# facebookresearch/goliath

Measured on AMD Instinct MI355X. Metric: relit views/sec (fwd+bwd) at 2048x1334, 250k Gaussians, higher is better.
Workload: dtype f32; 1 GPU; rgca_config2_envrelight; gaussians=250000, views_per_gpu=8, micro_batches=2, world_size=1, dist_backend=none, rccl_world_size=0, parallelism=view-parallel x1, launch=hip_graph_replay

## Files before the change

### goliath_amd/csrc/gol_raster.h

```cpp
#pragma once
#include <type_traits>

#include "gol_common.h"

namespace {

constexpr int kBatch = 256;
constexpr float kUnA = GOL_UN_A, kUnB = GOL_UN_B;
__device__ __forceinline__ float3 true_conic(float a, float b, float c) { return make_float3(a * kUnA, b * kUnB, c * kUnA); }
#ifdef GOL_EXACT_MATH
__device__ __forceinline__ float exact_sigma(float a, float b, float c, float dx, float dy) {
#pragma clang fp contract(off)
  const float t1 = (a * dx) * dx, t2 = (c * dy) * dy, t3 = (b * dx) * dy;
  const float h = 0.5f * (t1 + t2);
  return h + t3;
}
__device__ __forceinline__ float exact_exp_neg(float s) { return (float)exp(-(double)s); }
__device__ __forceinline__ float exact_next_T(float T, float alpha) {
#pragma clang fp contract(off)
  const float om = 1.f - alpha;
  return T * om;
}
#endif

struct TileCoord { int tile, tx, ty; bool ok; };

__device__ __forceinline__ TileCoord tile_of_block(int bid, int T, int tiles_x) {
  const int tiles_y = T / tiles_x;
  const int xcd = bid & 7, j = bid >> 3;
  TileCoord tc;
  const int row_local = j / tiles_x;
  tc.tx = j - row_local * tiles_x;
  tc.ty = row_local * 8 + xcd;
  tc.ok = tc.ty < tiles_y;
  tc.tile = tc.ty * tiles_x + tc.tx;
  return tc;
}

typedef float f1 __attribute__((ext_vector_type(1)));
typedef float f2 __attribute__((ext_vector_type(2)));
typedef int i1 __attribute__((ext_vector_type(1)));
typedef int i2 __attribute__((ext_vector_type(2)));

template <int PPL> struct Pix;
template <> struct Pix<2> { typedef f2 fv; typedef i2 iv; static constexpr int kWaves = 2; };
template <> struct Pix<1> { typedef f1 fv; typedef i1 iv; static constexpr int kWaves = 4; };

template <int PPL>
__device__ __forceinline__ void wave_rect(int wave, float tile_x0, float tile_y0, float& x0, float& x1, float& y0, float& y1) {
  if (PPL == 2) {
    x0 = tile_x0 + 0.5f; x1 = x0 + 15.f; y0 = tile_y0 + (float)(wave * 8) + 0.5f; y1 = y0 + 7.f;
  } else {
    x0 = tile_x0 + (float)((wave & 1) * 8) + 0.5f; x1 = x0 + 7.f; y0 = tile_y0 + (float)((wave >> 1) * 8) + 0.5f; y1 = y0 + 7.f;
  }
}

template <int PPL>
__device__ __forceinline__ int wave_mask(float gx, float gy, float ca, float cb, float cc, float tau, float ia, float ic,
                                         float exact, float tile_x0, float tile_y0) {
  constexpr int NW = Pix<PPL>::kWaves;
  if (!(tau >= 0.f)) return 0;
  if (exact == 0.f) return (1 << NW) - 1;
  int m = 0;
#pragma unroll
  for (int q = 0; q < NW; ++q) {
    float x0, x1, y0, y1;
    wave_rect<PPL>(q, tile_x0, tile_y0, x0, x1, y0, y1);
    const float ms = gol_min_sigma_rect(gx, gy, ca, cb, cc, ia, ic, x0, x1, y0, y1);
    m |= (ms <= tau) ? (1 << q) : 0;
  }
  return m;
}

template <int PPL>
__device__ __forceinline__ void lane_pixel(int tx, int ty, int wave, int lane, int& j, int& i0) {
  if (PPL == 2) { j = tx * 16 + (lane & 15); i0 = ty * 16 + wave * 8 + (lane >> 4) * 2; }
  else { j = tx * 16 + (wave & 1) * 8 + (lane & 7); i0 = ty * 16 + (wave >> 1) * 8 + (lane >> 3); }
}

struct __attribute__((aligned(16))) StagedRow { float4 a, b; float2 c; float2 pad; };

struct Staged { float4 a, b; float2 c; int mask; };
template <int PPL>
__device__ __forceinline__ Staged stage_entry(const float* __restrict__ records, size_t g, float tile_x0, float tile_y0) {
  const float4* R = reinterpret_cast<const float4*>(records + g * GOL_SPLAT_RECORD);
  const float4 q0 = R[0], q1 = R[1], q2 = R[2], q3 = R[3];
  Staged s;
  s.a = q0;
  s.b = q1;
  s.c = make_float2(q2.x, q2.y);
  const float3 cn = true_conic(q0.z, q0.w, q1.x);
  s.mask = wave_mask<PPL>(q0.x, q0.y, cn.x, cn.y, cn.z, q2.z, q2.w, q3.x, q3.y, tile_x0, tile_y0);
  return s;
}

template <typename V, int P>
__device__ __forceinline__ bool any_live(const V& live) {
  unsigned u = 0u;
#pragma unroll
  for (int q = 0; q < P; ++q) u |= __float_as_uint(live[q]);
  return u != 0u;
}

template <int PPL> using fvec = typename Pix<PPL>::fv;
template <int PPL> using ivec = typename Pix<PPL>::iv;

template <int PPL>
__device__ __forceinline__ void visit_falloff(float ca, float cb, float cc, float dx, const fvec<PPL>& dy, fvec<PPL>& sigma,
                                              fvec<PPL>& e) {
#ifndef GOL_EXACT_MATH
  sigma = (ca * dx * dx + cc * dy * dy) + (cb * dx) * dy;
#pragma unroll
  for (int q = 0; q < PPL; ++q) e[q] = __builtin_amdgcn_exp2f(-sigma[q]);
#else
#pragma unroll
  for (int q = 0; q < PPL; ++q) { sigma[q] = exact_sigma(ca, cb, cc, dx, dy[q]); e[q] = exact_exp_neg(sigma[q]); }
#endif
}

template <int PPL>
__device__ __forceinline__ unsigned long long fwd_step(const fvec<PPL>& sigma, fvec<PPL> alpha, const fvec<PPL>& live,
                                                       const fvec<PPL>& T_cur, fvec<PPL>& vis, fvec<PPL>& next_T,
                                                       bool (&take)[PPL], unsigned long long (&stop)[PPL]) {
  alpha *= live;
  vis = alpha * T_cur;
#ifndef GOL_EXACT_MATH
  next_T = T_cur - vis;
#else
#pragma unroll
  for (int q = 0; q < PPL; ++q) next_T[q] = exact_next_T(T_cur[q], alpha[q]);
#endif
  unsigned long long any_stop = 0ull;
#pragma unroll
  for (int q = 0; q < PPL; ++q) {
    const unsigned long long mc = gol_ballot(!(sigma[q] < 0.f)) & gol_ballot(!(alpha[q] < GOL_ALPHA_FLOOR));
    const unsigned long long ms = gol_ballot(next_T[q] <= GOL_T_STOP);
    take[q] = __builtin_amdgcn_inverse_ballot_w64(mc & ~ms);
    stop[q] = mc & ms;
    any_stop |= stop[q];
  }
  return any_stop;
}

template <int PPL>
__device__ __forceinline__ void fwd_take(const bool (&take)[PPL], const fvec<PPL>& next_T, fvec<PPL>& vis, fvec<PPL>& T_cur) {
#pragma unroll
  for (int q = 0; q < PPL; ++q) vis[q] = take[q] ? vis[q] : 0.f;
#ifndef GOL_EXACT_MATH
  T_cur -= vis;
#else
#pragma unroll
  for (int q = 0; q < PPL; ++q) T_cur[q] = take[q] ? next_T[q] : T_cur[q];
#endif
}

template <int PPL>
__device__ __forceinline__ unsigned long long bwd_taken(float opacity, const fvec<PPL>& e, const fvec<PPL>& sigma, int li,
                                                        const ivec<PPL>& bin_final, fvec<PPL>& alpha,
                                                        unsigned long long (&mv)[PPL]) {
  alpha = opacity * e;
  unsigned long long many = 0ull;
#pragma unroll
  for (int q = 0; q < PPL; ++q) {
    alpha[q] = fminf(GOL_ALPHA_CAP_BWD, alpha[q]);
    mv[q] = gol_ballot(li <= bin_final[q]) & gol_ballot(!(sigma[q] < 0.f)) & gol_ballot(!(alpha[q] < GOL_ALPHA_FLOOR));
    many |= mv[q];
  }
  return many;
}

template <int PPL>
__device__ __forceinline__ void bwd_recur(const unsigned long long (&mv)[PPL], fvec<PPL>& alpha, fvec<PPL>& T_cur,
                                          bool (&v)[PPL], fvec<PPL>& ra, fvec<PPL>& fac) {
#pragma unroll
  for (int q = 0; q < PPL; ++q) {
    v[q] = __builtin_amdgcn_inverse_ballot_w64(mv[q]);
    alpha[q] = v[q] ? alpha[q] : 0.f;
  }
  const fvec<PPL> one_m = 1.f - alpha;
#pragma unroll
  for (int q = 0; q < PPL; ++q) ra[q] = __builtin_amdgcn_rcpf(one_m[q]);
  const fvec<PPL> T_new = T_cur * ra;
  fac = alpha * T_new;
  T_cur = T_new;
}

template <int PPL>
__device__ __forceinline__ void bwd_moments(const fvec<PPL>& e, const fvec<PPL>& w, const fvec<PPL>& T_cur,
                                            const fvec<PPL>& ra, const fvec<PPL>& fac, const fvec<PPL>& tail,
                                            const bool (&v)[PPL], const fvec<PPL>& dy, fvec<PPL>& qsum, fvec<PPL>& gop,
                                            fvec<PPL>& gy, fvec<PPL>& gyy) {
  const fvec<PPL> v_alpha = T_cur * w + ra * (tail - qsum);
  qsum += fac * w;
  gop = e * v_alpha;
#pragma unroll
  for (int q = 0; q < PPL; ++q) gop[q] = v[q] ? gop[q] : 0.f;
  gy = gop * dy;
  gyy = gy * dy;
}
template <int PPL>
__device__ __forceinline__ float lane_sum(const fvec<PPL>& x) {
  float s = x[0];
#pragma unroll
  for (int q = 1; q < PPL; ++q) s += x[q];
  return s;
}

template <int PPL>
__device__ __forceinline__ int wave_last_entry(const ivec<PPL>& bin_final) {
  int wmax = bin_final[0];
#pragma unroll
  for (int q = 1; q < PPL; ++q) wmax = max(wmax, bin_final[q]);
#pragma unroll
  for (int off = 32; off > 0; off >>= 1) wmax = max(wmax, __shfl_xor(wmax, off, 64));
  return __builtin_amdgcn_readfirstlane(wmax);
}

inline int64_t raster_grid(int B, int img_h, int img_w) {
  return (int64_t)B * 8 * (((img_h + 15) / 16 + 7) / 8) * ((img_w + 15) / 16);
}

#define GOL_RASTER_CHECK_DIMS(bytes_per_pixel, too_large_msg)                                                           \
  do {                                                                                                                  \
    GOL_REQUIRE(B >= 0 && N >= 0, "negative size");                                                                     \
    GOL_REQUIRE(block == 16, "only block_width == 16 is implemented (the reference's value, render_gsplat.py:28)");     \
    GOL_REQUIRE(img_h > 0 && img_w > 0, "empty image");                                                                 \
    GOL_REQUIRE(raster_grid(B, img_h, img_w) < (1ll << 31), "too many tiles");                                          \
    GOL_REQUIRE((uint64_t)img_h * (uint64_t)img_w * (uint64_t)(bytes_per_pixel) < (1ull << 32), too_large_msg);         \
  } while (0)

template <typename F>
inline void with_ppl(int ppl, F&& fn) {
  if (ppl == 2) fn(std::integral_constant<int, 2>());
  else fn(std::integral_constant<int, 1>());
}
constexpr std::true_type kYes{}; constexpr std::false_type kNo{};

}
```

### goliath_amd/csrc/raster.hip

```cpp
#include <cstdlib>

#include "gol_raster.h"

namespace {

constexpr int kBgGroup = 4;

template <bool EXTRA, bool LAZY, int PPL>
__global__ __launch_bounds__(64 * Pix<PPL>::kWaves) void raster_fwd_kernel(
    int N, int img_h, int img_w, int planar, int tiles_x, int tiles_y, const int2* __restrict__ tile_bins,
    const int32_t* __restrict__ sorted_ids, int64_t capacity, const float* __restrict__ records,
    const float* __restrict__ background, float* __restrict__ out_img,
    float* __restrict__ out_extra, float* __restrict__ final_Ts, int32_t* __restrict__ final_idx,
    float* __restrict__ out_alpha, float* __restrict__ out_extra_norm, float norm_lo,
    const float* __restrict__ l1_target, const float* __restrict__ l1_mask, int l1_mask_c,
    uint8_t* __restrict__ l1_sign, float* __restrict__ l1_partial, int n_views, int bg_group, int bg_vec16) {
  typedef typename Pix<PPL>::fv fv;
  typedef typename Pix<PPL>::iv iv;
  constexpr int NW = Pix<PPL>::kWaves, NT = 64 * NW;
  __shared__ float s_l1[NW];
  __shared__ float4 s_a[kBatch];
  __shared__ float4 s_b[kBatch];
  __shared__ float2 s_c[kBatch];
  __shared__ int32_t s_mask[kBatch];
  const int T = tiles_x * tiles_y;
  const int view = blockIdx.x % n_views, slot = blockIdx.x / n_views;
  const TileCoord tc = tile_of_block(slot, T, tiles_x);
  if (!tc.ok) return;
  const int tid = threadIdx.x, lane = tid & 63, wave = tid >> 6;

  int2 range;
  auto fill_group = [&](auto g_c) -> bool {
    constexpr int G = decltype(g_c)::value;
    const int tx0 = tc.tx & ~(G - 1), n = min(G, tiles_x - tx0);
    const size_t tile0 = (size_t)view * T + (size_t)(tc.tile - (tc.tx - tx0));
    int entries = 0;
#pragma unroll
    for (int t = 0; t < G; ++t) {
      const int2 r = tile_bins[tile0 + min(t, n - 1)];
      entries |= (r.y > r.x) ? 1 : 0;
      if (t == tc.tx - tx0) range = r;
    }
    if (entries) return false;
    if (tc.tx != tx0) return true;
    const unsigned hw = (unsigned)img_h * (unsigned)img_w;
    const size_t vplane = (size_t)view * hw;
    const float Tq = 1.f, ex = 0.f;
    const float c0 = 0.f + Tq * background[0], c1 = 0.f + Tq * background[1], c2 = 0.f + Tq * background[2];
    const float al = 1.f - Tq;
    const float nrm = ex / fminf(fmaxf(1.f - Tq, norm_lo), 1.f);
    float* __restrict__ o_T = final_Ts + vplane;
    float* __restrict__ o_img = out_img + 3 * vplane;
    float* __restrict__ o_img1 = o_img + hw;
    float* __restrict__ o_img2 = o_img + 2u * hw;
    float* __restrict__ o_ex = (EXTRA && out_extra) ? out_extra + vplane : nullptr;
    float* __restrict__ o_alpha = out_alpha ? out_alpha + vplane : nullptr;
    float* __restrict__ o_norm = (EXTRA && out_extra_norm) ? out_extra_norm + vplane : nullptr;
    const int x0 = tx0 * 16, y0 = tc.ty * 16;
    const int rw = min(x0 + 16 * G, img_w) - x0, nrows = min(16, img_h - y0);
    auto fill_rows = [&](auto v_c) {
      constexpr int V = decltype(v_c)::value;
      typedef float vt __attribute__((ext_vector_type(V)));
      typedef int it __attribute__((ext_vector_type(V)));
      constexpr int CPR = 16 * G / V, RPP = NT / CPR;
      const int col = (tid % CPR) * V, r0 = tid / CPR;
#pragma unroll
      for (int k = 0; k * RPP < 16; ++k) {
        const int r = r0 + k * RPP;
        if (col < rw && r < nrows) {
          const unsigned b4 = ((unsigned)(y0 + r) * (unsigned)img_w + (unsigned)(x0 + col)) * 4u;
          *reinterpret_cast<vt*>(gol_at(o_T, b4)) = vt(Tq);
          if (!LAZY) *reinterpret_cast<it*>(gol_at(final_idx + vplane, b4)) = it(0);
          *reinterpret_cast<vt*>(gol_at(o_img, b4)) = vt(c0);
          *reinterpret_cast<vt*>(gol_at(o_img1, b4)) = vt(c1);
          *reinterpret_cast<vt*>(gol_at(o_img2, b4)) = vt(c2);
          if (o_ex) *reinterpret_cast<vt*>(gol_at(o_ex, b4)) = vt(ex);
          if (o_alpha) *reinterpret_cast<vt*>(gol_at(o_alpha, b4)) = vt(al);
          if (o_norm) *reinterpret_cast<vt*>(gol_at(o_norm, b4)) = vt(nrm);
        }
      }
    };
    if (bg_vec16) fill_rows(std::integral_constant<int, 4>());
    else fill_rows(std::integral_constant<int, 2>());
    if (!l1_target) return true;
    const float* __restrict__ i_tgt = l1_target + 3 * vplane;
    const float* __restrict__ i_mask = l1_mask ? l1_mask + (size_t)l1_mask_c * vplane : nullptr;
    float* s_part = reinterpret_cast<float*>(s_a);
    constexpr int CH = G < 4 ? G : 4;
    auto l1_tiles = [&](auto m_c) {
      constexpr int MC = decltype(m_c)::value;
      const float cs[3] = {c0, c1, c2};
#pragma unroll
      for (int tb = 0; tb < G; tb += CH) {
        if (tb >= n) break;
        float tg[CH][PPL][3], mk[CH][PPL][3];
        bool ok[CH][PPL];
#pragma unroll
        for (int t = 0; t < CH; ++t) {
          int tj, ti0;
          lane_pixel<PPL>(tx0 + tb + t, tc.ty, wave, lane, tj, ti0);
#pragma unroll
          for (int q = 0; q < PPL; ++q) {
            ok[t][q] = (ti0 + q < img_h) && (tj < img_w);
            const unsigned b4 = ((unsigned)min(ti0 + q, img_h - 1) * (unsigned)img_w + (unsigned)min(tj, img_w - 1)) * 4u;
#pragma unroll
            for (int c = 0; c < 3; ++c) {
              tg[t][q][c] = *gol_at(i_tgt + (size_t)c * hw, b4);
              mk[t][q][c] = MC == 0 ? 1.f : (MC == 3 || c == 0) ? *gol_at(i_mask + (size_t)c * hw, b4) : mk[t][q][0];
            }
          }
        }
#pragma unroll
        for (int t = 0; t < CH; ++t) {
          float l1_acc = 0.f;
#pragma unroll
          for (int q = 0; q < PPL; ++q) {
#pragma unroll
            for (int c = 0; c < 3; ++c) {
              const float d = (cs[c] - tg[t][q][c]) * mk[t][q][c];
              l1_acc += ok[t][q] ? fabsf(d) : 0.f;
            }
          }
          const float ws = gol_wave_sum_to_lane63(l1_acc);
          if (lane == 63) s_part[(tb + t) * NW + wave] = ws;
        }
      }
    };
    if (!i_mask) l1_tiles(std::integral_constant<int, 0>());
    else if (l1_mask_c == 3) l1_tiles(std::integral_constant<int, 3>());
    else l1_tiles(std::integral_constant<int, 1>());
    __syncthreads();
    if (tid < n) {
      float tot = 0.f;
#pragma unroll
      for (int w = 0; w < NW; ++w) tot += s_part[tid * NW + w];
      l1_partial[tile0 + tid] = tot;
    }
    return true;
  };
  if (PPL == 2 && bg_group) {
    const bool done = bg_group == 2 ? fill_group(std::integral_constant<int, 2>())
                    : bg_group == 4 ? fill_group(std::integral_constant<int, 4>())
                                    : fill_group(std::integral_constant<int, 8>());
    if (done) return;
  } else {
    range = tile_bins[(size_t)view * T + tc.tile];
  }

  int j, i0;
  lane_pixel<PPL>(tc.tx, tc.ty, wave, lane, j, i0);
  bool in[PPL];
  fv py, live;
#pragma unroll
  for (int q = 0; q < PPL; ++q) {
    in[q] = (i0 + q < img_h) && (j < img_w);
    py[q] = (float)(i0 + q) + 0.5f;
    live[q] = in[q] ? 1.f : 0.f;
  }
  const float px = (float)j + 0.5f;

  const int32_t* ids = sorted_ids + (size_t)view * capacity;
  const size_t goff = (size_t)view * N;

  fv T_cur = 1.f;
  iv cur_idx = 0;
  fv acc0 = 0.f, acc1 = 0.f, acc2 = 0.f, acc3 = 0.f;

  const int n_batches = (range.y - range.x + kBatch - 1) / kBatch;
  for (int bb = 0; bb < n_batches; ++bb) {
    if (__syncthreads_and(!any_live<fv, PPL>(live))) break;
    const int batch_start = range.x + bb * kBatch;
    for (int k = tid; k < kBatch; k += NT) {
      const int idx = batch_start + k;
      if (idx < range.y) {
        const Staged st = stage_entry<PPL>(records, goff + (size_t)ids[idx], (float)(tc.tx * 16), (float)(tc.ty * 16));
        s_a[k] = st.a; s_b[k] = st.b; s_c[k] = st.c; s_mask[k] = st.mask;
      } else {
        s_mask[k] = 0;
      }
    }
    __syncthreads();
    const int batch_size = min(kBatch, range.y - batch_start);
    for (int chunk = 0; chunk < batch_size; chunk += 64) {
      unsigned long long bits = gol_ballot((s_mask[chunk + lane] >> wave) & 1);
      if (LAZY && gol_ballot(any_live<fv, PPL>(live)) == 0ull) break;
      while (bits) {
        if (!LAZY && gol_ballot(any_live<fv, PPL>(live)) == 0ull) { chunk = batch_size; break; }
        const int t = chunk + __builtin_ctzll(bits);
        bits &= bits - 1;
        const float4 a4 = s_a[t];
        const float4 b4 = s_b[t];
        const float2 c2 = s_c[t];
        const float dx = a4.x - px;
        const fv dy = a4.y - py;
        fv sigma, e, alpha, vis, next_T;
        visit_falloff<PPL>(a4.z, a4.w, b4.x, dx, dy, sigma, e);
#pragma unroll
        for (int q = 0; q < PPL; ++q) alpha[q] = fminf(GOL_ALPHA_CAP_FWD, b4.y * e[q]);
        bool take[PPL];
        unsigned long long stop_m[PPL];
        const unsigned long long any_stop = fwd_step<PPL>(sigma, alpha, live, T_cur, vis, next_T, take, stop_m);
        bool half_done = false;
        if (!LAZY || any_stop != 0ull) {
#pragma unroll
          for (int q = 0; q < PPL; ++q) {
            const bool stop = __builtin_amdgcn_inverse_ballot_w64(stop_m[q]);
            live[q] = stop ? 0.f : live[q];
            if (LAZY) cur_idx[q] = stop ? (batch_start + t - 1) : cur_idx[q];
          }
          if (LAZY) half_done = gol_ballot(any_live<fv, PPL>(live)) == 0ull;
        }
        fwd_take<PPL>(take, next_T, vis, T_cur);
        acc0 += b4.z * vis; acc1 += b4.w * vis; acc2 += c2.x * vis;
        if (EXTRA) acc3 += c2.y * vis;
        if (!LAZY) {
#pragma unroll
          for (int q = 0; q < PPL; ++q) cur_idx[q] = take[q] ? (batch_start + t) : cur_idx[q];
        }
        if (LAZY && half_done) { chunk = batch_size; break; }
      }
    }
  }
  if (LAZY) {
#pragma unroll
    for (int q = 0; q < PPL; ++q) cur_idx[q] = live[q] != 0.f ? range.y - 1 : cur_idx[q];
  }

  const unsigned hw = (unsigned)img_h * (unsigned)img_w;
  const size_t vplane = (size_t)view * hw;
  float* __restrict__ o_T = final_Ts + vplane;
  int32_t* __restrict__ o_idx = final_idx + vplane;
  float* __restrict__ o_img = out_img + 3 * vplane;
  float* __restrict__ o_ex = (EXTRA && out_extra) ? out_extra + vplane : nullptr;
  float* __restrict__ o_alpha = out_alpha ? out_alpha + vplane : nullptr;
  float* __restrict__ o_norm = (EXTRA && out_extra_norm) ? out_extra_norm + vplane : nullptr;
  const float* __restrict__ i_tgt = l1_target ? l1_target + 3 * vplane : nullptr;
  const float* __restrict__ i_mask = l1_mask ? l1_mask + (size_t)l1_mask_c * vplane : nullptr;
  uint8_t* __restrict__ o_sign = l1_target ? l1_sign + vplane : nullptr;
  const float bg0 = background[0], bg1 = background[1], bg2 = background[2];
  float* __restrict__ o_img1 = o_img + (planar ? hw : 1u);
  float* __restrict__ o_img2 = o_img + (planar ? 2u * hw : 2u);
  const bool bwd_state = range.y > range.x;
  float l1_acc = 0.f;
#pragma unroll
  for (int q = 0; q < PPL; ++q) {
    if (!in[q]) continue;
    const unsigned pix = (unsigned)(i0 + q) * (unsigned)img_w + (unsigned)j;
    const unsigned b4 = pix * 4u;
    const unsigned bimg = planar ? b4 : 3u * b4;
    const float Tq = T_cur[q];
    const float c0 = acc0[q] + Tq * bg0, c1 = acc1[q] + Tq * bg1, c2 = acc2[q] + Tq * bg2, ex = acc3[q];
    *gol_at(o_T, b4) = Tq;
    if (bwd_state || !LAZY) *gol_at(o_idx, b4) = cur_idx[q];
    *gol_at(o_img, bimg) = c0; *gol_at(o_img1, bimg) = c1; *gol_at(o_img2, bimg) = c2;
    if (o_ex) *gol_at(o_ex, b4) = ex;
    if (o_alpha) *gol_at(o_alpha, b4) = 1.f - Tq;
    if (o_norm) *gol_at(o_norm, b4) = ex / fminf(fmaxf(1.f - Tq, norm_lo), 1.f);
    if (i_tgt) {
      const float m0 = i_mask ? *gol_at(i_mask, b4) : 1.f;
      const float cs[3] = {c0, c1, c2};
      unsigned code = 0u;
#pragma unroll
      for (int c = 0; c < 3; ++c) {
        const float m = (i_mask && l1_mask_c == 3) ? *gol_at(i_mask + (size_t)c * hw, b4) : m0;
        const float d = (cs[c] - *gol_at(i_tgt + (size_t)c * hw, b4)) * m;
        l1_acc += fabsf(d);
        code |= (d > 0.f ? 2u : (d < 0.f ? 0u : 1u)) << (2 * c);
      }
      if (bwd_state) *gol_at(o_sign, pix) = (uint8_t)code;
    }
  }
  if (l1_target) {
    const float ws = gol_wave_sum_to_lane63(l1_acc);
    if (lane == 63) s_l1[wave] = ws;
    __syncthreads();
    if (tid == 0) {
      float tot = 0.f;
#pragma unroll
      for (int w = 0; w < NW; ++w) tot += s_l1[w];
      l1_partial[(size_t)view * T + tc.tile] = tot;
    }
  }
}

__global__ __launch_bounds__(1024) void l1_sum_kernel(int n, const float* __restrict__ l1_partial, float scale,
                                                      float* __restrict__ l1_out) {
  __shared__ float s_w[16];
  float a0 = 0.f, a1 = 0.f, a2 = 0.f, a3 = 0.f;
  const int n4 = n >> 2;
  const float4* p4 = reinterpret_cast<const float4*>(l1_partial);
  int i = threadIdx.x;
  for (; i + 3 * 1024 < n4; i += 4 * 1024) {
    const float4 v0 = p4[i], v1 = p4[i + 1024], v2 = p4[i + 2048], v3 = p4[i + 3072];
    a0 += (v0.x + v0.y) + (v0.z + v0.w); a1 += (v1.x + v1.y) + (v1.z + v1.w);
    a2 += (v2.x + v2.y) + (v2.z + v2.w); a3 += (v3.x + v3.y) + (v3.z + v3.w);
  }
  for (; i < n4; i += 1024) { const float4 v = p4[i]; a0 += (v.x + v.y) + (v.z + v.w); }
  if ((int)threadIdx.x < (n & 3)) a1 += l1_partial[4 * n4 + threadIdx.x];
  const float ws = gol_wave_sum_to_lane63((a0 + a1) + (a2 + a3));
  if ((threadIdx.x & 63) == 63) s_w[threadIdx.x >> 6] = ws;
  __syncthreads();
  if (threadIdx.x == 0) {
    float tot = 0.f;
#pragma unroll
    for (int w = 0; w < 16; ++w) tot += s_w[w];
    l1_out[0] = tot * scale;
  }
}

constexpr int kBatchB = 64;
constexpr int kAcc = 12;

static_assert(kBatchB == 64, "raster_bwd_kernel ballots one 64-entry chunk per batch");

template <bool EXTRA, bool PACKED, int PPL>
__global__ __launch_bounds__(64 * Pix<PPL>::kWaves) void raster_bwd_kernel(
    int N, int img_h, int img_w, int planar, int tiles_x, int tiles_y, const int2* __restrict__ tile_bins,
    const int32_t* __restrict__ sorted_ids, int64_t capacity, const float* __restrict__ records,
    const float* __restrict__ background,
    const float* __restrict__ final_Ts, const int32_t* __restrict__ final_idx,
    const float* __restrict__ v_out_img, const float* __restrict__ v_out_extra,
    const float* __restrict__ v_out_alpha, float* __restrict__ v_xy, float* __restrict__ v_conic,
    float* __restrict__ v_colors, float* __restrict__ v_extra, float* __restrict__ v_opacity,
    const uint8_t* __restrict__ v_sign, const float* __restrict__ v_sign_mask, int v_sign_mask_c,
    const float* __restrict__ v_img_scale, float v_img_scale_mul, int n_views) {
  typedef typename Pix<PPL>::fv fv;
  typedef typename Pix<PPL>::iv iv;
  constexpr int NW = Pix<PPL>::kWaves, NT = 64 * NW;
  __shared__ StagedRow s_e[kBatchB];
  __shared__ int32_t s_mask[kBatchB];
  __shared__ int32_t s_id[kBatchB];
  __shared__ __attribute__((aligned(16))) float s_acc[NW][kBatchB][kAcc];
  __shared__ int32_t s_touched[NW][kBatchB];
  __shared__ int32_t s_wmax[NW];
  const int T = tiles_x * tiles_y;
  const int view = blockIdx.x % n_views, slot = blockIdx.x / n_views;
  const TileCoord tc = tile_of_block(slot, T, tiles_x);
  if (!tc.ok) return;
  const int2 range = tile_bins[(size_t)view * T + tc.tile];
  if (range.y <= range.x) return;
  const int tid = threadIdx.x, lane = tid & 63, wave = tid >> 6;
  int j, i0;
  lane_pixel<PPL>(tc.tx, tc.ty, wave, lane, j, i0);
  const float px = (float)j + 0.5f;
  const size_t hw = (size_t)img_h * img_w;
  const int32_t* ids = sorted_ids + (size_t)view * capacity;
  const size_t goff = (size_t)view * N;
  bool in[PPL];
  size_t pp[PPL];
  fv py, T_final;
  iv bin_final;
#pragma unroll
  for (int q = 0; q < PPL; ++q) {
    in[q] = (i0 + q < img_h) && (j < img_w);
    py[q] = (float)(i0 + q) + 0.5f;
    pp[q] = in[q] ? ((size_t)view * img_h + i0 + q) * img_w + j : 0;
    T_final[q] = in[q] ? final_Ts[pp[q]] : 1.f;
    bin_final[q] = in[q] ? final_idx[pp[q]] : (range.x - 1);
  }
  fv T_cur = T_final;
  fv vo0 = 0.f, vo1 = 0.f, vo2 = 0.f, vo3 = 0.f, voa = 0.f;
  {
    const float vsc = (v_img_scale ? v_img_scale[0] : 1.f) * v_img_scale_mul;
    const size_t os = planar ? hw : 1;
#pragma unroll
    for (int q = 0; q < PPL; ++q) {
      if (!in[q]) continue;
      const size_t p = pp[q];
      const int i = i0 + q;
      const size_t o = planar ? (size_t)view * 3 * hw + (size_t)i * img_w + j : 3 * p;
      float g0 = 0.f, g1 = 0.f, g2 = 0.f;
      if (v_out_img) { g0 = v_out_img[o]; g1 = v_out_img[o + os]; g2 = v_out_img[o + 2 * os]; }
      if (v_sign) {
        const unsigned code = v_sign[p];
        float m0 = vsc, m1 = vsc, m2 = vsc;
        if (v_sign_mask) {
          const float* mk = v_sign_mask + (size_t)view * v_sign_mask_c * hw + (size_t)i * img_w + j;
          m0 *= mk[0]; m1 *= (v_sign_mask_c == 3) ? mk[hw] : mk[0]; m2 *= (v_sign_mask_c == 3) ? mk[2 * hw] : mk[0];
        }
        g0 += (float)((int)(code & 3u) - 1) * m0;
        g1 += (float)((int)((code >> 2) & 3u) - 1) * m1;
        g2 += (float)((int)((code >> 4) & 3u) - 1) * m2;
      }
      vo0[q] = g0; vo1[q] = g1; vo2[q] = g2;
      if (EXTRA && v_out_extra) vo3[q] = v_out_extra[p];
      if (v_out_alpha) voa[q] = v_out_alpha[p];
    }
  }
  const fv tail = T_final * (voa - (background[0] * vo0 + background[1] * vo1 + background[2] * vo2));
  fv qsum = 0.f;

  const int wmax = wave_last_entry<PPL>(bin_final);
  if (lane == 0) s_wmax[wave] = wmax;
  __syncthreads();
  int bmax = s_wmax[0];
#pragma unroll
  for (int w = 1; w < NW; ++w) bmax = max(bmax, s_wmax[w]);
  bmax = min(bmax, range.y - 1);
  if (bmax < range.x) return;

  float* acc_lane = &s_acc[wave][0][lane >> 4];
  const int n_batches = (bmax - range.x + kBatchB) / kBatchB;
  auto entry_id = [&](int bb2) {
    const int e = bmax - bb2 * kBatchB - tid;
    return (tid < kBatchB && e >= range.x) ? ids[e] : 0;
  };
  int gid_next = entry_id(0);
  unsigned rec_bytes = GOL_GRAD_RECORD * sizeof(float);
  if (PACKED) asm volatile("" : "+s"(rec_bytes));
  for (int bb = 0; bb < n_batches; ++bb) {
    __syncthreads();
    const int batch_end = bmax - bb * kBatchB;
    const int batch_size = min(kBatchB, batch_end + 1 - range.x);
    const int gid = gid_next;
    if (tid < kBatchB) {
      if (tid < batch_size) {
        const Staged st = stage_entry<PPL>(records, goff + (size_t)gid, (float)(tc.tx * 16), (float)(tc.ty * 16));
        s_e[tid].a = st.a; s_e[tid].b = st.b; s_e[tid].c = st.c; s_mask[tid] = st.mask;
        s_id[tid] = gid;
      } else {
        s_mask[tid] = 0;
      }
    }
    if (bb + 1 < n_batches) gid_next = entry_id(bb + 1);
    (&s_touched[0][0])[tid] = 0;
    __syncthreads();

    const int t0 = max(0, batch_end - wmax);
    unsigned long long bits = gol_ballot((s_mask[lane] >> wave) & 1);
    if (t0 > 0) bits &= ~0ull << t0;
    while (bits) {
      const int t = __builtin_ctzll(bits);
      bits &= bits - 1;
      const float4 a4 = s_e[t].a;
      const float4 b4 = s_e[t].b;
      const float2 c2 = s_e[t].c;
      const int li = batch_end - t;
      const float dx = a4.x - px;
      const fv dy = a4.y - py;
      fv sigma, vis, alpha, ra, fac;
      visit_falloff<PPL>(a4.z, a4.w, b4.x, dx, dy, sigma, vis);
      unsigned long long mv[PPL];
      if (bwd_taken<PPL>(b4.y, vis, sigma, li, bin_final, alpha, mv) == 0ull) continue;
      bool v[PPL];
      bwd_recur<PPL>(mv, alpha, T_cur, v, ra, fac);
      fv w = b4.z * vo0 + b4.w * vo1 + c2.x * vo2;
      if (EXTRA) w += c2.y * vo3;
      fv gop, gy, gyy;
      bwd_moments<PPL>(vis, w, T_cur, ra, fac, tail, v, dy, qsum, gop, gy, gyy);
      float g0s, g1s, g2s, g3 = 0.f;
      if (PPL == 2) {
        g0s = __builtin_fmaf(fac[0], vo0[0], fac[PPL - 1] * vo0[PPL - 1]);
        g1s = __builtin_fmaf(fac[0], vo1[0], fac[PPL - 1] * vo1[PPL - 1]);
        g2s = __builtin_fmaf(fac[0], vo2[0], fac[PPL - 1] * vo2[PPL - 1]);
        if (EXTRA) g3 = __builtin_fmaf(fac[0], vo3[0], fac[PPL - 1] * vo3[PPL - 1]);
      } else {
        g0s = fac[0] * vo0[0]; g1s = fac[0] * vo1[0]; g2s = fac[0] * vo2[0];
        if (EXTRA) g3 = fac[0] * vo3[0];
      }
      const float m0 = lane_sum<PPL>(gop), my = lane_sum<PPL>(gy), myy = lane_sum<PPL>(gyy);
      const float mx = m0 * dx, mxx = mx * dx, mxy = my * dx;
      const float r0 = gol_wave_sum4(g0s, g1s, g2s, m0);
      const float r1 = gol_wave_sum4(mx, my, mxx, mxy);
      const float r2 = gol_wave_sum_to_lane63(myy);
      const float r3 = EXTRA ? gol_wave_sum_to_lane63(g3) : 0.f;
      if ((lane & 15) == 15) {
        float* a = gol_at(acc_lane, (unsigned)t * (unsigned)(kAcc * sizeof(float)));
        a[0] = r0; a[4] = r1;
        if (lane == 63) { a[8 - 3] = r2; a[9 - 3] = r3; }
        s_touched[wave][t] = 1;
      }
    }
    __syncthreads();
    if (PACKED) {
      if (tid < kBatchB) {
        int tw[NW];
#pragma unroll
        for (int w = 0; w < NW; ++w) tw[w] = s_touched[w][tid];
        float s[kAcc];
#pragma unroll
        for (int k = 0; k < kAcc; ++k) s[k] = 0.f;
        bool any = false;
#pragma unroll
        for (int w = 0; w < NW; ++w) {
          if (tw[w]) {
            any = true;
            const float4* q = reinterpret_cast<const float4*>(&s_acc[w][tid][0]);
            const float4 q0 = q[0], q1 = q[1], q2 = q[2];
            s[0] += q0.x; s[1] += q0.y; s[2] += q0.z; s[3] += q0.w;
            s[4] += q1.x; s[5] += q1.y; s[6] += q1.z; s[7] += q1.w;
            s[8] += q2.x; s[9] += q2.y;
          }
        }
        if (any) {
          const float4 a4 = s_e[tid].a;
          const float4 b4 = s_e[tid].b;
          const float nop = -b4.y, cc = b4.x;
          const float wxx = nop * a4.z * kUnA, wxy = nop * a4.w * kUnB, wyy = nop * cc * kUnA, hnop = 0.5f * nop;
          float4* o = reinterpret_cast<float4*>(&s_acc[0][tid][0]);
          o[0] = make_float4(s[0], s[1], s[2], s[3]);
          o[1] = make_float4(wxx * s[4] + wxy * s[5], wxy * s[4] + wyy * s[5], hnop * s[6], nop * s[7]);
          *reinterpret_cast<float2*>(o + 2) = make_float2(hnop * s[8], s[9]);
          s_touched[0][tid] = 1;
        }
      }
      __syncthreads();
      const int c = tid & 15;
      if (c <= (EXTRA ? 9 : 8)) {
        float* rec_c = v_colors + goff * 16 + c;
        constexpr int kIt = kBatchB * 16 / NT, kCh = 4;
        static_assert(kIt % kCh == 0, "the merge issues its atomics in chunks of kCh entries per lane");
#pragma unroll
        for (int i0 = 0; i0 < kIt; i0 += kCh) {
          int flag[kCh], id[kCh];
          float val[kCh];
#pragma unroll
          for (int i = 0; i < kCh; ++i) {
            const int t = (tid >> 4) + (i0 + i) * (NT / 16);
            flag[i] = s_touched[0][t]; id[i] = s_id[t]; val[i] = s_acc[0][t][c];
          }
#pragma unroll
          for (int i = 0; i < kCh; ++i) {
            if (flag[i]) {
              char* r = reinterpret_cast<char*>(rec_c) + (uint64_t)(unsigned)id[i] * rec_bytes;
              atomicAdd(reinterpret_cast<float*>(r), val[i]);
            }
          }
        }
      }
    } else if (tid < batch_size) {
      float a[kAcc];
#pragma unroll
      for (int k = 0; k < kAcc; ++k) a[k] = 0.f;
      bool any = false;
#pragma unroll
      for (int w = 0; w < NW; ++w) {
        if (s_touched[w][tid]) {
          any = true;
          const float4* q = reinterpret_cast<const float4*>(&s_acc[w][tid][0]);
          const float4 q0 = q[0], q1 = q[1], q2 = q[2];
          a[0] += q0.x; a[1] += q0.y; a[2] += q0.z; a[3] += q0.w;
          a[4] += q1.x; a[5] += q1.y; a[6] += q1.z; a[7] += q1.w;
          a[8] += q2.x; a[9] += q2.y;
        }
      }
      if (any) {
        const size_t g = goff + (size_t)s_id[tid];
        const float4 a4 = s_e[tid].a;
        const float4 b4 = s_e[tid].b;
        const float nop = -b4.y;
        const float3 cn = true_conic(a4.z, a4.w, b4.x);
        atomicAdd(v_colors + 3 * g, a[0]); atomicAdd(v_colors + 3 * g + 1, a[1]); atomicAdd(v_colors + 3 * g + 2, a[2]);
        atomicAdd(v_opacity + g, a[3]);
        atomicAdd(v_xy + 2 * g, nop * (cn.x * a[4] + cn.y * a[5]));
        atomicAdd(v_xy + 2 * g + 1, nop * (cn.y * a[4] + cn.z * a[5]));
        atomicAdd(v_conic + 3 * g, 0.5f * nop * a[6]); atomicAdd(v_conic + 3 * g + 1, nop * a[7]);
        atomicAdd(v_conic + 3 * g + 2, 0.5f * nop * a[8]);
        if (EXTRA && v_extra) atomicAdd(v_extra + g, a[9]);
      }
    }
  }
}

__global__ __launch_bounds__(256) void raster_count_pairs_kernel(int N, int img_h, int img_w, int tiles_x, int tiles_y,
                                                                 const int2* __restrict__ tile_bins,
                                                                 const int32_t* __restrict__ sorted_ids, int64_t capacity,
                                                                 const float* __restrict__ records,
                                                                 const int32_t* __restrict__ final_idx,
                                                                 unsigned long long* __restrict__ counts) {
  __shared__ unsigned long long s_cnt[2];
  const int view = blockIdx.y, tile = blockIdx.x, T = tiles_x * tiles_y;
  const int ty = tile / tiles_x, tx = tile - ty * tiles_x;
  const int j = tx * 16 + (threadIdx.x & 15), i = ty * 16 + (threadIdx.x >> 4);
  if (threadIdx.x < 2) s_cnt[threadIdx.x] = 0ull;
  __syncthreads();
  const int2 range = tile_bins[(size_t)view * T + tile];
  unsigned long long tested = 0, taken = 0;
  if (i < img_h && j < img_w && range.y > range.x) {
    const int last = min(range.y - 1, final_idx[((size_t)view * img_h + i) * img_w + j]);
    const float px = (float)j + 0.5f, py = (float)i + 0.5f;
    for (int li = range.x; li <= last; ++li) {
      const float4* R = reinterpret_cast<const float4*>(records + ((size_t)view * N + sorted_ids[(size_t)view * capacity + li]) * GOL_SPLAT_RECORD);
      const float4 q0 = R[0], q1 = R[1];
      const float dx = q0.x - px, dy = q0.y - py;
      f1 sg, e;
      visit_falloff<1>(q0.z, q0.w, q1.x, dx, f1(dy), sg, e);
      const float alpha = fminf(GOL_ALPHA_CAP_FWD, q1.y * e[0]);
      ++tested;
      taken += (!(sg[0] < 0.f) && !(alpha < GOL_ALPHA_FLOOR)) ? 1 : 0;
    }
  }
  atomicAdd(&s_cnt[0], tested);
  atomicAdd(&s_cnt[1], taken);
  __syncthreads();
  if (threadIdx.x < 2 && s_cnt[threadIdx.x]) atomicAdd(counts + 2 * view + threadIdx.x, s_cnt[threadIdx.x]);
}

__global__ __launch_bounds__(256) void splat_pack_kernel(size_t n, const float* __restrict__ xys,
                                                         const float* __restrict__ conics,
                                                         const float* __restrict__ colors,
                                                         const float* __restrict__ extra,
                                                         const float* __restrict__ opacities,
                                                         float* __restrict__ records) {
  const size_t e = (size_t)blockIdx.x * 256 + threadIdx.x;
  if (e >= n) return;
  gol_record_write(records + e * GOL_SPLAT_RECORD, xys[2 * e], xys[2 * e + 1], conics[3 * e], conics[3 * e + 1],
                   conics[3 * e + 2], opacities[e], colors ? colors[3 * e] : 0.f, colors ? colors[3 * e + 1] : 0.f,
                   colors ? colors[3 * e + 2] : 0.f, extra ? extra[e] : 0.f);
}

}

extern "C" int gol_raster_plan(int B, int* fwd_pixels_per_lane) {
  static const int forced = getenv("GOL_RASTER_PPL") ? atoi(getenv("GOL_RASTER_PPL")) : 0;
  if (fwd_pixels_per_lane) *fwd_pixels_per_lane = (forced == 1 || forced == 2) ? forced : (B <= 2 ? 1 : 2);
  return GOL_OK;
}

extern "C" int gol_raster_count_pairs(int B, int N, int img_h, int img_w, const int32_t* tile_bins, const int32_t* sorted_ids,
                                      int64_t capacity, const float* records, const int32_t* final_idx, uint64_t* counts,
                                      void* stream) {
  GOL_REQUIRE(B >= 0 && N >= 0 && img_h > 0 && img_w > 0, "bad size");
  if (B == 0) return GOL_OK;
  GOL_REQUIRE(tile_bins && final_idx && counts && (capacity == 0 || sorted_ids) && (N == 0 || records), "null pointer");
  hipStream_t s = (hipStream_t)stream;
  if (hipMemsetAsync(counts, 0, sizeof(uint64_t) * 2 * (size_t)B, s) != hipSuccess) {
    gol_set_error("gol_raster_count_pairs: hipMemsetAsync failed");
    return GOL_ERR_LAUNCH;
  }
  const int tiles_x = (img_w + 15) / 16, tiles_y = (img_h + 15) / 16;
  raster_count_pairs_kernel<<<dim3(tiles_x * tiles_y, B), 256, 0, s>>>(
      N, img_h, img_w, tiles_x, tiles_y, reinterpret_cast<const int2*>(tile_bins), sorted_ids, capacity, records, final_idx,
      reinterpret_cast<unsigned long long*>(counts));
  GOL_CHECK_LAUNCH();
  return GOL_OK;
}

extern "C" int gol_splat_pack(int B, int N, const float* xys, const float* conics, const float* colors,
                              const float* extra, const float* opacities, float* records, void* stream) {
  GOL_REQUIRE(B >= 0 && N >= 0, "negative size");
  if (B == 0 || N == 0) return GOL_OK;
  GOL_REQUIRE(xys && conics && opacities && records, "null pointer");
  const size_t n = (size_t)B * N;
  splat_pack_kernel<<<gol_cdiv((long long)n, 256), 256, 0, (hipStream_t)stream>>>(n, xys, conics, colors, extra, opacities,
                                                                                 records);
  GOL_CHECK_LAUNCH();
  return GOL_OK;
}

extern "C" int gol_rasterize_fwd(int B, int N, int img_h, int img_w, int block, int planar, const int32_t* tile_bins,
                                 const int32_t* sorted_ids, int64_t capacity, const float* records, int with_extra,
                                 const float* background, float* out_img,
                                 float* out_extra, float* final_Ts, int32_t* final_idx, float* out_alpha,
                                 float* out_extra_norm, float norm_lo, const float* l1_target, const float* l1_mask,
                                 int l1_mask_c, uint8_t* l1_sign, float* l1_partial, float* l1_out, float l1_scale,
                                 int pixels_per_lane, void* stream) {
  GOL_RASTER_CHECK_DIMS(12, "image too large (32-bit byte offsets inside a view)");
  if (B == 0) return GOL_OK;
  GOL_REQUIRE(tile_bins && background && out_img && final_Ts && final_idx, "null pointer");
  GOL_REQUIRE(capacity == 0 || sorted_ids, "null sorted_ids");
  GOL_REQUIRE(N == 0 || records, "null Gaussian records");
  GOL_REQUIRE((!out_extra && !out_extra_norm) || with_extra || N == 0, "out_extra / out_extra_norm need the extra channel");
  GOL_REQUIRE(!with_extra || out_extra || out_extra_norm, "extra without an output for it");
  GOL_REQUIRE(!l1_target || (planar && l1_sign && l1_partial), "the fused L1 needs planar images, l1_sign and l1_partial");
  GOL_REQUIRE(!l1_mask || (l1_target && (l1_mask_c == 1 || l1_mask_c == 3)), "l1_mask: 1 or 3 channels, with l1_target");
  GOL_REQUIRE(!l1_out || l1_target, "l1_out needs l1_target");
  const int tiles_x = (img_w + 15) / 16, tiles_y = (img_h + 15) / 16;
  const dim3 grid((unsigned)raster_grid(B, img_h, img_w));
  const int2* bins = reinterpret_cast<const int2*>(tile_bins);
  hipStream_t s = (hipStream_t)stream;
  GOL_REQUIRE(pixels_per_lane >= 0 && pixels_per_lane <= 2, "pixels_per_lane: 0 (choose by B), 1 or 2");
  int ppl = pixels_per_lane;
  if (ppl == 0) gol_raster_plan(B, &ppl);
  int bg_group = kBgGroup, bg_vec16 = 0;
  if (const char* e = getenv("GOL_RASTER_BG_GROUP")) bg_group = atoi(e);
  GOL_REQUIRE(bg_group == 0 || bg_group == 2 || bg_group == 4 || bg_group == 8, "GOL_RASTER_BG_GROUP: 0, 2, 4 or 8");
  if (!planar || (img_w & 1) || ppl != 2) bg_group = 0;
  if (bg_group) {
    uintptr_t bits = 0;
    for (const void* p : {(const void*)out_img, (const void*)final_Ts, (const void*)out_extra, (const void*)out_alpha,
                          (const void*)out_extra_norm})
      bits |= reinterpret_cast<uintptr_t>(p);
    bg_vec16 = (img_w % 4 == 0 && bits % 16 == 0) ? 1 : 0;
    if (bits % 8 != 0) bg_group = 0;
  }
  auto launch = [&](auto ex_c, auto lazy_c) {
    with_ppl(ppl, [&](auto ppl_c) {
      constexpr bool EX = decltype(ex_c)::value, LZ = decltype(lazy_c)::value;
      constexpr int PPL = decltype(ppl_c)::value;
      raster_fwd_kernel<EX, LZ, PPL><<<grid, 64 * Pix<PPL>::kWaves, 0, s>>>(
          N, img_h, img_w, planar, tiles_x, tiles_y, bins, sorted_ids, capacity, records, background, out_img, out_extra,
          final_Ts, final_idx, out_alpha, EX ? out_extra_norm : nullptr, norm_lo, l1_target, l1_mask, l1_mask_c, l1_sign,
          l1_partial, B, bg_group, bg_vec16);
    });
  };
  const bool ex = out_extra || out_extra_norm;
  if (ex && planar) launch(kYes, kYes);
  else if (ex) launch(kYes, kNo);
  else if (planar) launch(kNo, kYes);
  else launch(kNo, kNo);
  if (l1_out) l1_sum_kernel<<<1, 1024, 0, s>>>(B * tiles_x * tiles_y, l1_partial, l1_scale, l1_out);
  GOL_CHECK_LAUNCH();
  return GOL_OK;
}

extern "C" int gol_rasterize_bwd(int B, int N, int img_h, int img_w, int block, int planar, const int32_t* tile_bins,
                                 const int32_t* sorted_ids, int64_t capacity, const float* records, int with_extra,
                                 const float* background, const float* final_Ts,
                                 const int32_t* final_idx, const float* v_out_img, const float* v_out_extra,
                                 const float* v_out_alpha, float* v_xy, float* v_conic, float* v_colors,
                                 float* v_extra, float* v_opacity, int grad_stride, const uint8_t* v_sign,
                                 const float* v_sign_mask, int v_sign_mask_c, const float* v_img_scale,
                                 float v_img_scale_mul, int pixels_per_lane, void* stream) {
  GOL_RASTER_CHECK_DIMS(0, "");
  if (B == 0 || N == 0 || capacity == 0) return GOL_OK;
  GOL_REQUIRE(tile_bins && sorted_ids && background && final_Ts && final_idx, "null pointer");
  GOL_REQUIRE(v_out_img || v_sign, "no upstream image gradient (v_out_img or v_sign)");
  GOL_REQUIRE(!v_sign || planar, "the sign image of the fused L1 goes with planar images");
  GOL_REQUIRE(!v_sign_mask || (v_sign && (v_sign_mask_c == 1 || v_sign_mask_c == 3)), "v_sign_mask: 1 or 3 channels, with v_sign");
  GOL_REQUIRE(records, "null Gaussian records");
  GOL_REQUIRE(v_xy && v_conic && v_colors && v_opacity, "null gradient output");
  GOL_REQUIRE(!(v_out_extra || v_extra) || with_extra, "extra-channel gradients need the extra channel");
  GOL_REQUIRE(grad_stride == 0 || grad_stride == GOL_GRAD_RECORD, "grad_stride must be 0 (dense arrays) or 16 (records)");
  const bool packed = grad_stride == GOL_GRAD_RECORD;
  if (packed)
    GOL_REQUIRE(v_opacity == v_colors + 3 && v_xy == v_colors + 4 && v_conic == v_colors + 6 &&
                    (!v_extra || v_extra == v_colors + 9),
                "record layout is [rgb | opacity | xy | conic | extra | pad] (GOL_GRAD_RECORD floats)");
  const int tiles_x = (img_w + 15) / 16, tiles_y = (img_h + 15) / 16;
  const dim3 grid((unsigned)raster_grid(B, img_h, img_w));
  const int2* bins = reinterpret_cast<const int2*>(tile_bins);
  hipStream_t s = (hipStream_t)stream;
  GOL_REQUIRE(pixels_per_lane >= 0 && pixels_per_lane <= 2, "pixels_per_lane: 0 (2), 1 or 2");
  const int ppl = pixels_per_lane ? pixels_per_lane : 2;
  const bool ex = with_extra && (v_out_extra || v_extra);
  auto launch = [&](auto ex_c, auto packed_c) {
    with_ppl(ppl, [&](auto ppl_c) {
      constexpr bool EX = decltype(ex_c)::value, PK = decltype(packed_c)::value;
      constexpr int PPL = decltype(ppl_c)::value;
      raster_bwd_kernel<EX, PK, PPL><<<grid, 64 * Pix<PPL>::kWaves, 0, s>>>(
          N, img_h, img_w, planar, tiles_x, tiles_y, bins, sorted_ids, capacity, records, background, final_Ts, final_idx,
          v_out_img, EX ? v_out_extra : nullptr, v_out_alpha, v_xy, v_conic, v_colors, EX ? v_extra : nullptr, v_opacity,
          v_sign, v_sign_mask, v_sign_mask_c, v_img_scale, v_img_scale_mul, B);
    });
  };
  if (ex && packed) launch(kYes, kYes);
  else if (ex) launch(kYes, kNo);
  else if (packed) launch(kNo, kYes);
  else launch(kNo, kNo);
  GOL_CHECK_LAUNCH();
  return GOL_OK;
}
```

### goliath_amd/csrc/raster_nd.hip

```cpp
#include "gol_raster.h"

namespace {

constexpr int kChunkMax = 16;
constexpr int kBatchNdB = 64;

template <int CK>
__device__ __forceinline__ void stage_colors(float* __restrict__ row, const float* __restrict__ colors, size_t g, int C,
                                             int c0, int nc) {
  const float* col = colors + g * (size_t)C + c0;
#pragma unroll
  for (int c = 0; c < CK; ++c) row[c] = (c < nc) ? col[c] : 0.f;
}

template <int CK, int PPL>
__global__ __launch_bounds__(64 * Pix<PPL>::kWaves) void raster_nd_fwd_kernel(
    int N, int C, int c_first, int img_h, int img_w, int tiles_x, int tiles_y, const int2* __restrict__ tile_bins,
    const int32_t* __restrict__ sorted_ids, int64_t capacity, const float* __restrict__ records,
    const float* __restrict__ colors, const float* __restrict__ background, float* __restrict__ out_img,
    float* __restrict__ final_Ts, int32_t* __restrict__ final_idx, int n_views) {
  typedef typename Pix<PPL>::fv fv;
  typedef typename Pix<PPL>::iv iv;
  constexpr int NW = Pix<PPL>::kWaves, NT = 64 * NW;
  __shared__ float4 s_a[kBatch];
  __shared__ float2 s_b[kBatch];
  __shared__ int32_t s_mask[kBatch];
  __shared__ __attribute__((aligned(16))) float s_col[kBatch * CK];
  const int T = tiles_x * tiles_y;
  const int view = blockIdx.x % n_views, slot = blockIdx.x / n_views;
  const TileCoord tc = tile_of_block(slot, T, tiles_x);
  if (!tc.ok) return;
  const int c0 = c_first + (int)blockIdx.y * CK;
  const int nc = min(CK, C - c0);
  const int tid = threadIdx.x, lane = tid & 63, wave = tid >> 6;
  int j, i0;
  lane_pixel<PPL>(tc.tx, tc.ty, wave, lane, j, i0);
  bool in[PPL];
  fv py, live;
#pragma unroll
  for (int q = 0; q < PPL; ++q) {
    in[q] = (i0 + q < img_h) && (j < img_w);
    py[q] = (float)(i0 + q) + 0.5f;
    live[q] = in[q] ? 1.f : 0.f;
  }
  const float px = (float)j + 0.5f;

  const int2 range = tile_bins[(size_t)view * T + tc.tile];
  const int32_t* ids = sorted_ids + (size_t)view * capacity;
  const size_t goff = (size_t)view * N;

  fv T_cur = 1.f;
  iv cur_idx = 0;
  fv acc[CK];
#pragma unroll
  for (int c = 0; c < CK; ++c) acc[c] = 0.f;

  const int n_batches = (range.y - range.x + kBatch - 1) / kBatch;
  for (int bb = 0; bb < n_batches; ++bb) {
    if (__syncthreads_and(!any_live<fv, PPL>(live))) break;
    const int batch_start = range.x + bb * kBatch;
    for (int k = tid; k < kBatch; k += NT) {
      const int idx = batch_start + k;
      if (idx < range.y) {
        const size_t g = goff + (size_t)ids[idx];
        const Staged st = stage_entry<PPL>(records, g, (float)(tc.tx * 16), (float)(tc.ty * 16));
        s_a[k] = st.a; s_b[k] = make_float2(st.b.x, st.b.y); s_mask[k] = st.mask;
        stage_colors<CK>(s_col + k * CK, colors, g, C, c0, nc);
      } else {
        s_mask[k] = 0;
      }
    }
    __syncthreads();
    const int batch_size = min(kBatch, range.y - batch_start);
    for (int chunk = 0; chunk < batch_size; chunk += 64) {
      unsigned long long bits = gol_ballot((s_mask[chunk + lane] >> wave) & 1);
      while (bits) {
        if (gol_ballot(any_live<fv, PPL>(live)) == 0ull) { chunk = batch_size; break; }
        const int t = chunk + __builtin_ctzll(bits);
        bits &= bits - 1;
        const float4 a4 = s_a[t];
        const float2 b2 = s_b[t];
        const float dx = a4.x - px;
        const fv dy = a4.y - py;
        fv sigma, e, alpha, vis, next_T;
        visit_falloff<PPL>(a4.z, a4.w, b2.x, dx, dy, sigma, e);
#pragma unroll
        for (int q = 0; q < PPL; ++q) alpha[q] = fminf(GOL_ALPHA_CAP_FWD, b2.y * e[q]);
        bool take[PPL];
        unsigned long long stop_m[PPL];
        fwd_step<PPL>(sigma, alpha, live, T_cur, vis, next_T, take, stop_m);
#pragma unroll
        for (int q = 0; q < PPL; ++q) live[q] = __builtin_amdgcn_inverse_ballot_w64(stop_m[q]) ? 0.f : live[q];
        fwd_take<PPL>(take, next_T, vis, T_cur);
        const float* col = s_col + t * CK;
#pragma unroll
        for (int c = 0; c < CK; ++c) acc[c] += col[c] * vis;
#pragma unroll
        for (int q = 0; q < PPL; ++q) cur_idx[q] = take[q] ? (batch_start + t) : cur_idx[q];
      }
    }
  }

  const unsigned hw = (unsigned)img_h * (unsigned)img_w;
  const size_t vplane = (size_t)view * hw;
  float* __restrict__ o_img = out_img + (size_t)C * vplane + c0;
  float* __restrict__ o_T = final_Ts + vplane;
  int32_t* __restrict__ o_idx = final_idx + vplane;
  const bool first = c0 == 0;
  float bg[CK];
#pragma unroll
  for (int c = 0; c < CK; ++c) bg[c] = (c < nc) ? background[c0 + c] : 0.f;
#pragma unroll
  for (int q = 0; q < PPL; ++q) {
    if (!in[q]) continue;
    const unsigned pix = (unsigned)(i0 + q) * (unsigned)img_w + (unsigned)j;
    const float Tq = T_cur[q];
    if (first) { *gol_at(o_T, pix * 4u) = Tq; *gol_at(o_idx, pix * 4u) = cur_idx[q]; }
    const unsigned bimg = pix * (unsigned)C * 4u;
#pragma unroll
    for (int c = 0; c < CK; ++c)
      if (c < nc) *gol_at(o_img + c, bimg) = acc[c][q] + Tq * bg[c];
  }
}

template <int CK, int PPL>
__global__ __launch_bounds__(64 * Pix<PPL>::kWaves) void raster_nd_bwd_kernel(
    int N, int C, int c_first, int img_h, int img_w, int tiles_x, int tiles_y, const int2* __restrict__ tile_bins,
    const int32_t* __restrict__ sorted_ids, int64_t capacity, const float* __restrict__ records,
    const float* __restrict__ colors, const float* __restrict__ background, const float* __restrict__ final_Ts,
    const int32_t* __restrict__ final_idx, const float* __restrict__ v_out_img, const float* __restrict__ v_out_alpha,
    float* __restrict__ v_xy, float* __restrict__ v_conic, float* __restrict__ v_colors, float* __restrict__ v_opacity,
    int n_views) {
  typedef typename Pix<PPL>::fv fv;
  typedef typename Pix<PPL>::iv iv;
  constexpr int NW = Pix<PPL>::kWaves, NT = 64 * NW;
  constexpr int NS = CK + 6, NG = (NS + 3) / 4, kRow = 4 * NG;
  static_assert(NW * kBatchNdB == NT, "s_touched is cleared one element per thread");
  __shared__ float4 s_a[kBatchNdB];
  __shared__ float2 s_b[kBatchNdB];
  __shared__ int32_t s_mask[kBatchNdB];
  __shared__ int32_t s_id[kBatchNdB];
  __shared__ __attribute__((aligned(16))) float s_col[kBatchNdB * CK];
  __shared__ __attribute__((aligned(16))) float s_acc[NW][kBatchNdB][kRow];
  __shared__ int32_t s_touched[NW][kBatchNdB];
  __shared__ int32_t s_wmax[NW];
  const int T = tiles_x * tiles_y;
  const int view = blockIdx.x % n_views, slot = blockIdx.x / n_views;
  const TileCoord tc = tile_of_block(slot, T, tiles_x);
  if (!tc.ok) return;
  const int2 range = tile_bins[(size_t)view * T + tc.tile];
  if (range.y <= range.x) return;
  const int c0 = c_first + (int)blockIdx.y * CK;
  const int nc = min(CK, C - c0);
  const int tid = threadIdx.x, lane = tid & 63, wave = tid >> 6;
  int j, i0;
  lane_pixel<PPL>(tc.tx, tc.ty, wave, lane, j, i0);
  const float px = (float)j + 0.5f;
  const int32_t* ids = sorted_ids + (size_t)view * capacity;
  const size_t goff = (size_t)view * N;
  fv py, T_final, voa = 0.f;
  iv bin_final;
  fv vo[CK];
#pragma unroll
  for (int c = 0; c < CK; ++c) vo[c] = 0.f;
#pragma unroll
  for (int q = 0; q < PPL; ++q) {
    const bool in = (i0 + q < img_h) && (j < img_w);
    py[q] = (float)(i0 + q) + 0.5f;
    const size_t p = in ? ((size_t)view * img_h + i0 + q) * img_w + j : 0;
    T_final[q] = in ? final_Ts[p] : 1.f;
    bin_final[q] = in ? final_idx[p] : (range.x - 1);
    if (in) {
      const float* g = v_out_img + p * (size_t)C + c0;
#pragma unroll
      for (int c = 0; c < CK; ++c) vo[c][q] = (c < nc) ? g[c] : 0.f;
      if (v_out_alpha && c0 == 0) voa[q] = v_out_alpha[p];
    }
  }

  const int wmax = wave_last_entry<PPL>(bin_final);
  if (lane == 0) s_wmax[wave] = wmax;
  __syncthreads();
  int bmax = s_wmax[0];
#pragma unroll
  for (int w = 1; w < NW; ++w) bmax = max(bmax, s_wmax[w]);
  bmax = min(bmax, range.y - 1);
  if (bmax < range.x) return;

  fv bgdot = 0.f;
#pragma unroll
  for (int c = 0; c < CK; ++c) bgdot += ((c < nc) ? background[c0 + c] : 0.f) * vo[c];
  const fv tail = T_final * (voa - bgdot);
  fv T_cur = T_final;
  fv qsum = 0.f;

  float* acc_lane = &s_acc[wave][0][lane >> 4];
  const int n_batches = (bmax - range.x + kBatchNdB) / kBatchNdB;
  for (int bb = 0; bb < n_batches; ++bb) {
    __syncthreads();
    const int batch_end = bmax - bb * kBatchNdB;
    const int batch_size = min(kBatchNdB, batch_end + 1 - range.x);
    if (tid < kBatchNdB) {
      if (tid < batch_size) {
        const int gid = ids[batch_end - tid];
        const size_t g = goff + (size_t)gid;
        const Staged st = stage_entry<PPL>(records, g, (float)(tc.tx * 16), (float)(tc.ty * 16));
        s_a[tid] = st.a; s_b[tid] = make_float2(st.b.x, st.b.y); s_mask[tid] = st.mask;
        s_id[tid] = gid;
        stage_colors<CK>(s_col + tid * CK, colors, g, C, c0, nc);
      } else {
        s_mask[tid] = 0;
      }
    }
    (&s_touched[0][0])[tid] = 0;
    __syncthreads();

    const int t0 = max(0, batch_end - wmax);
    unsigned long long bits = gol_ballot((s_mask[lane] >> wave) & 1);
    if (t0 > 0) bits &= ~0ull << t0;
    while (bits) {
      const int t = __builtin_ctzll(bits);
      bits &= bits - 1;
      const float4 a4 = s_a[t];
      const float2 b2 = s_b[t];
      const int li = batch_end - t;
      const float dx = a4.x - px;
      const fv dy = a4.y - py;
      fv sigma, vis, alpha, ra, fac;
      visit_falloff<PPL>(a4.z, a4.w, b2.x, dx, dy, sigma, vis);
      unsigned long long mv[PPL];
      if (bwd_taken<PPL>(b2.y, vis, sigma, li, bin_final, alpha, mv) == 0ull) continue;
      bool v[PPL];
      bwd_recur<PPL>(mv, alpha, T_cur, v, ra, fac);
      const float* col = s_col + t * CK;
      fv w = 0.f;
#pragma unroll
      for (int c = 0; c < CK; ++c) w += col[c] * vo[c];
      fv gop, gy, gyy;
      bwd_moments<PPL>(vis, w, T_cur, ra, fac, tail, v, dy, qsum, gop, gy, gyy);
      float s[kRow];
#pragma unroll
      for (int c = 0; c < CK; ++c) {
        s[c] = fac[0] * vo[c][0];
#pragma unroll
        for (int q = 1; q < PPL; ++q) s[c] = __builtin_fmaf(fac[q], vo[c][q], s[c]);
      }
      const float m0 = lane_sum<PPL>(gop), my = lane_sum<PPL>(gy), myy = lane_sum<PPL>(gyy);
      const float mx = m0 * dx;
      s[CK + 0] = m0; s[CK + 1] = mx; s[CK + 2] = my; s[CK + 3] = mx * dx; s[CK + 4] = my * dx; s[CK + 5] = myy;
#pragma unroll
      for (int k = NS; k < kRow; ++k) s[k] = 0.f;
      float r[NG];
#pragma unroll
      for (int gi = 0; gi < NG; ++gi) r[gi] = gol_wave_sum4(s[4 * gi], s[4 * gi + 1], s[4 * gi + 2], s[4 * gi + 3]);
      if ((lane & 15) == 15) {
        float* a = gol_at(acc_lane, (unsigned)t * (unsigned)(kRow * sizeof(float)));
#pragma unroll
        for (int gi = 0; gi < NG; ++gi) a[4 * gi] = r[gi];
        s_touched[wave][t] = 1;
      }
    }
    __syncthreads();
    for (int idx = tid; idx < batch_size * NS; idx += NT) {
      const int t = idx / NS, k = idx - t * NS;
      if (k < CK && k >= nc) continue;
      bool any = false;
#pragma unroll
      for (int w = 0; w < NW; ++w) any = any || (s_touched[w][t] != 0);
      if (!any) continue;
      const size_t g = goff + (size_t)s_id[t];
      const float4 a4 = s_a[t];
      const float2 b2 = s_b[t];
      const float nop = -b2.y;
      const float3 cn = true_conic(a4.z, a4.w, b2.x);
      const float ca = cn.x, cb = cn.y, cc = cn.z;
      int k1 = k, k2 = k;
      float w1 = 1.f, w2 = 0.f;
      float* dst;
      if (k < CK) {
        dst = v_colors + g * (size_t)C + c0 + k;
      } else {
        const int m = k - CK;
        k1 = (m == 1 || m == 2) ? CK + 1 : k;
        k2 = CK + 2;
        w1 = (m == 0) ? 1.f : (m == 1) ? nop * ca : (m == 2) ? nop * cb : (m == 4) ? nop : 0.5f * nop;
        w2 = (m == 1) ? nop * cb : (m == 2) ? nop * cc : 0.f;
        dst = (m == 0) ? v_opacity + g : (m <= 2) ? v_xy + 2 * g + (m - 1) : v_conic + 3 * g + (m - 3);
      }
      float s1 = 0.f, s2 = 0.f;
#pragma unroll
      for (int w = 0; w < NW; ++w) {
        const bool tw = s_touched[w][t] != 0;
        s1 += tw ? s_acc[w][t][k1] : 0.f;
        s2 += tw ? s_acc[w][t][k2] : 0.f;
      }
      atomicAdd(dst, w1 * s1 + w2 * s2);
    }
  }
}

struct NdPlan { int n16, tail, tail_first; };
NdPlan nd_plan(int C) {
  const int r = C % kChunkMax;
  NdPlan p;
  p.n16 = C / kChunkMax + (r > 8 ? 1 : 0);
  p.tail = (r == 0 || r > 8) ? 0 : r <= 1 ? 1 : r <= 2 ? 2 : r <= 4 ? 4 : 8;
  p.tail_first = (C / kChunkMax) * kChunkMax;
  return p;
}

template <typename F>
bool for_nd_launches(int C, F&& fn) {
  const NdPlan pl = nd_plan(C);
  if (pl.n16 > 0) fn(std::integral_constant<int, 16>(), pl.n16, 0);
  switch (pl.tail) {
    case 0: break;
    case 1: fn(std::integral_constant<int, 1>(), 1, pl.tail_first); break;
    case 2: fn(std::integral_constant<int, 2>(), 1, pl.tail_first); break;
    case 4: fn(std::integral_constant<int, 4>(), 1, pl.tail_first); break;
    case 8: fn(std::integral_constant<int, 8>(), 1, pl.tail_first); break;
    default: return false;
  }
  return true;
}

}

extern "C" int gol_rasterize_nd_fwd(int B, int N, int C, int img_h, int img_w, int block, const int32_t* tile_bins,
                                    const int32_t* sorted_ids, int64_t capacity, const float* records, const float* colors,
                                    const float* background, float* out_img, float* final_Ts, int32_t* final_idx,
                                    int pixels_per_lane, void* stream) {
  GOL_REQUIRE(C >= 1, "C >= 1 colour channels");
  GOL_REQUIRE(C <= 16 * 65535, "too many colour channels (at most 1048560: one launch row of 16-channel chunks)");
  GOL_RASTER_CHECK_DIMS((uint64_t)C * 4ull, "image too large (32-bit byte offsets inside a view: H * W * C * 4 bytes)");
  if (B == 0) return GOL_OK;
  GOL_REQUIRE(tile_bins && background && out_img && final_Ts && final_idx, "null pointer");
  GOL_REQUIRE(capacity == 0 || sorted_ids, "null sorted_ids");
  GOL_REQUIRE(N == 0 || (records && colors), "null Gaussian records / colors");
  GOL_REQUIRE(pixels_per_lane >= 0 && pixels_per_lane <= 2, "pixels_per_lane: 0 (choose by B), 1 or 2");
  int ppl = pixels_per_lane;
  if (ppl == 0) gol_raster_plan(B, &ppl);
  const int tiles_x = (img_w + 15) / 16, tiles_y = (img_h + 15) / 16;
  const unsigned gx = (unsigned)raster_grid(B, img_h, img_w);
  const int2* bins = reinterpret_cast<const int2*>(tile_bins);
  hipStream_t s = (hipStream_t)stream;
  const bool covered = for_nd_launches(C, [&](auto ck_c, int n_chunks, int c_first) {
    with_ppl(ppl, [&](auto ppl_c) {
      constexpr int CK = decltype(ck_c)::value, PPL = decltype(ppl_c)::value;
      raster_nd_fwd_kernel<CK, PPL><<<dim3(gx, n_chunks), 64 * Pix<PPL>::kWaves, 0, s>>>(
          N, C, c_first, img_h, img_w, tiles_x, tiles_y, bins, sorted_ids, capacity, records, colors, background, out_img,
          final_Ts, final_idx, B);
    });
  });
  GOL_REQUIRE(covered, "no kernel instance for this chunk width");
  GOL_CHECK_LAUNCH();
  return GOL_OK;
}

extern "C" int gol_rasterize_nd_bwd(int B, int N, int C, int img_h, int img_w, int block, const int32_t* tile_bins,
                                    const int32_t* sorted_ids, int64_t capacity, const float* records, const float* colors,
                                    const float* background, const float* final_Ts, const int32_t* final_idx,
                                    const float* v_out_img, const float* v_out_alpha, float* v_xy, float* v_conic,
                                    float* v_colors, float* v_opacity, void* stream) {
  GOL_REQUIRE(C >= 1, "C >= 1 colour channels");
  GOL_REQUIRE(C <= 16 * 65535, "too many colour channels (at most 1048560: one launch row of 16-channel chunks)");
  GOL_RASTER_CHECK_DIMS((uint64_t)C * 4ull, "image too large (32-bit byte offsets inside a view: H * W * C * 4 bytes)");
  if (B == 0 || N == 0 || capacity == 0) return GOL_OK;
  GOL_REQUIRE(tile_bins && sorted_ids && background && final_Ts && final_idx, "null pointer");
  GOL_REQUIRE(v_out_img, "null v_out_img");
  GOL_REQUIRE(records && colors, "null Gaussian records / colors");
  GOL_REQUIRE(v_xy && v_conic && v_colors && v_opacity, "null gradient output");
  const int tiles_x = (img_w + 15) / 16, tiles_y = (img_h + 15) / 16;
  const unsigned gx = (unsigned)raster_grid(B, img_h, img_w);
  const int2* bins = reinterpret_cast<const int2*>(tile_bins);
  hipStream_t s = (hipStream_t)stream;
  const bool covered = for_nd_launches(C, [&](auto ck_c, int n_chunks, int c_first) {
    constexpr int CK = decltype(ck_c)::value;
    raster_nd_bwd_kernel<CK, 2><<<dim3(gx, n_chunks), 128, 0, s>>>(
        N, C, c_first, img_h, img_w, tiles_x, tiles_y, bins, sorted_ids, capacity, records, colors, background, final_Ts,
        final_idx, v_out_img, v_out_alpha, v_xy, v_conic, v_colors, v_opacity, B);
  });
  GOL_REQUIRE(covered, "no kernel instance for this chunk width");
  GOL_CHECK_LAUNCH();
  return GOL_OK;
}
```

### goliath_amd/csrc/render.hip

```cpp
#include <cstring>

#include "gol_common.h"

namespace {
inline int64_t align256(int64_t x) { return (x + 255) & ~(int64_t)255; }
template <typename T>
inline T* at(void* ws, int64_t off) { return reinterpret_cast<T*>(reinterpret_cast<char*>(ws) + off); }
}

static int render_layout(int B, int N, int img_h, int img_w, int64_t capacity, int with_l1, bool projected, gol_render_ws* L) {
  GOL_REQUIRE(B >= 0 && N >= 0 && img_h > 0 && img_w > 0 && capacity >= 0 && L != nullptr, "bad argument");
  const int64_t T = (int64_t)((img_w + 15) / 16) * ((img_h + 15) / 16), P = (int64_t)img_h * img_w;
  const int64_t BN = (int64_t)B * N, cap = capacity > 0 ? capacity : 1;
  int64_t o = 0;
  auto take = [&](int64_t bytes) { const int64_t at_ = o; o = align256(o + bytes); return at_; };
  L->cov3d = -1;
  L->xys = projected ? -1 : take(BN * 2 * 4);
  L->depths = projected ? -1 : take(BN * 4);
  L->radii = projected ? -1 : take(BN * 4);
  L->conics = projected ? -1 : take(BN * 3 * 4);
  L->comp = projected ? -1 : take(BN * 4);
  L->nth = -1;
  L->opac_eff = projected ? -1 : take(BN * 4);
  L->records = projected ? -1 : take(BN * GOL_SPLAT_RECORD * 4);
  L->tile_count = take((int64_t)B * T * 4);
  L->tile_bins = take((int64_t)B * T * 2 * 4);
  L->keys = take((int64_t)B * cap * 8);
  L->sorted_ids = take((int64_t)B * cap * 4);
  L->n_isect = take((int64_t)B * 4);
  L->final_T = take((int64_t)B * P * 4);
  L->final_idx = take((int64_t)B * P * 4);
  L->l1_sign = with_l1 ? take((int64_t)B * P) : -1;
  L->total = o;
  return GOL_OK;
}

extern "C" int gol_render_layout(int B, int N, int img_h, int img_w, int64_t capacity, int with_l1, gol_render_ws* L) {
  return render_layout(B, N, img_h, img_w, capacity, with_l1, false, L);
}

extern "C" int gol_render_layout_projected(int B, int N, int img_h, int img_w, int64_t capacity, int with_l1,
                                           gol_render_ws* L) {
  return render_layout(B, N, img_h, img_w, capacity, with_l1, true, L);
}

static int render_fwd_from(int B, int N, int img_h, int img_w, const float* xys, const float* depths, const int32_t* radii,
                           const float* conics, const float* opac_eff, const float* records, const float* background,
                           int with_depth, float norm_lo, int64_t capacity, void* ws, const gol_render_ws* L,
                           float* out_img, float* out_depth, float* out_alpha, float* out_depth_norm,
                           const float* l1_target, const float* l1_mask, int l1_mask_c, float* l1_partial, float* l1_out,
                           float l1_scale, void* stream) {
  int rc = gol_bin_sort(B, N, xys, depths, radii, conics, opac_eff, img_h, img_w, 16, capacity,
                        at<int32_t>(ws, L->tile_count), at<int32_t>(ws, L->tile_bins), at<uint64_t>(ws, L->keys),
                        at<int32_t>(ws, L->sorted_ids), at<int32_t>(ws, L->n_isect), nullptr, stream);
  if (rc != GOL_OK) return rc;
  return gol_rasterize_fwd(B, N, img_h, img_w, 16, 1, at<int32_t>(ws, L->tile_bins), at<int32_t>(ws, L->sorted_ids),
                           capacity, records, with_depth ? 1 : 0, background, out_img,
                           with_depth ? out_depth : nullptr, at<float>(ws, L->final_T), at<int32_t>(ws, L->final_idx),
                           out_alpha, with_depth ? out_depth_norm : nullptr, norm_lo, l1_target, l1_mask, l1_mask_c,
                           l1_target ? at<uint8_t>(ws, L->l1_sign) : nullptr, l1_partial, l1_out, l1_scale, 0,
                           stream);
}

static int render_bwd_to_records(int B, int N, int img_h, int img_w, const float* records, const float* background,
                                 int64_t capacity, void* ws, const gol_render_ws* L, const float* v_img,
                                 const float* v_depth, const float* v_alpha, int use_l1_sign, const float* l1_mask,
                                 int l1_mask_c, const float* v_img_scale, float v_img_scale_mul, float* grad_records,
                                 void* stream) {
  hipStream_t s = (hipStream_t)stream;
  if (hipMemsetAsync(grad_records, 0, sizeof(float) * (size_t)B * N * GOL_GRAD_RECORD, s) != hipSuccess) {
    gol_set_error("gol_render_bwd: hipMemsetAsync failed");
    return GOL_ERR_LAUNCH;
  }
  float* g = grad_records;
  const bool use_depth = v_depth != nullptr;
  return gol_rasterize_bwd(B, N, img_h, img_w, 16, 1, at<int32_t>(ws, L->tile_bins), at<int32_t>(ws, L->sorted_ids),
                           capacity, records, use_depth ? 1 : 0, background,
                           at<float>(ws, L->final_T), at<int32_t>(ws, L->final_idx), v_img, v_depth, v_alpha, g + 4, g + 6,
                           g, use_depth ? g + 9 : nullptr, g + 3, GOL_GRAD_RECORD,
                           use_l1_sign ? at<uint8_t>(ws, L->l1_sign) : nullptr, use_l1_sign ? l1_mask : nullptr,
                           use_l1_sign ? l1_mask_c : 0, v_img_scale, v_img_scale_mul, 0, stream);
}

extern "C" int gol_render_fwd(int B, int N, int img_h, int img_w, float glob_scale, float clip_thresh, const float* means,
                              const float* scales, const float* quats, const float* opacity, const float* colors,
                              const float* viewmats, const float* intrins, const float* background, int with_depth,
                              float norm_lo, int64_t capacity, void* workspace, const gol_render_ws* L, float* out_img,
                              float* out_depth, float* out_alpha, float* out_depth_norm, const float* l1_target,
                              const float* l1_mask, int l1_mask_c, float* l1_partial, float* l1_out, float l1_scale,
                              void* stream) {
  GOL_REQUIRE(workspace != nullptr && L != nullptr, "null workspace / layout");
  GOL_REQUIRE(!l1_target || L->l1_sign >= 0, "layout was computed without the fused L1");
  if (B == 0) return GOL_OK;
  void* ws = workspace;
  GOL_REQUIRE(!l1_out || l1_target, "l1_out needs l1_target");
  int rc = gol_project_fwd(B, N, means, scales, glob_scale, quats, viewmats, intrins, img_h, img_w, 16, clip_thresh,
                           nullptr, at<float>(ws, L->xys), at<float>(ws, L->depths),
                           at<int32_t>(ws, L->radii), at<float>(ws, L->conics), at<float>(ws, L->comp),
                           nullptr, opacity, at<float>(ws, L->opac_eff), colors,
                           at<float>(ws, L->records), stream);
  if (rc != GOL_OK) return rc;
  return render_fwd_from(B, N, img_h, img_w, at<float>(ws, L->xys), at<float>(ws, L->depths), at<int32_t>(ws, L->radii),
                         at<float>(ws, L->conics), at<float>(ws, L->opac_eff), at<float>(ws, L->records), background,
                         with_depth, norm_lo, capacity, ws, L, out_img, out_depth, out_alpha, out_depth_norm, l1_target,
                         l1_mask, l1_mask_c, l1_partial, l1_out, l1_scale, stream);
}

extern "C" int gol_render_fwd_projected(int B, int N, const gol_shade_proj* proj, const float* background, int with_depth,
                                        float norm_lo, int64_t capacity, void* workspace, const gol_render_ws* L,
                                        float* out_img, float* out_depth, float* out_alpha, float* out_depth_norm,
                                        const float* l1_target, const float* l1_mask, int l1_mask_c, float* l1_partial,
                                        float* l1_out, float l1_scale, void* stream) {
  GOL_REQUIRE(workspace != nullptr && L != nullptr && proj != nullptr, "null workspace / layout / projection");
  GOL_REQUIRE(!l1_target || L->l1_sign >= 0, "layout was computed without the fused L1");
  GOL_REQUIRE(!l1_out || l1_target, "l1_out needs l1_target");
  if (B == 0) return GOL_OK;
  return render_fwd_from(B, N, proj->img_h, proj->img_w, proj->xys, proj->depths, proj->radii, proj->conics,
                         proj->opac_eff, proj->records, background, with_depth, norm_lo, capacity, workspace, L, out_img,
                         out_depth, out_alpha, out_depth_norm, l1_target, l1_mask, l1_mask_c, l1_partial, l1_out,
                         l1_scale, stream);
}

extern "C" int gol_render_bwd(int B, int N, int img_h, int img_w, float glob_scale, const float* means,
                              const float* scales, const float* quats, const float* opacity, const float* viewmats,
                              const float* intrins, const float* background, int64_t capacity, void* workspace,
                              const gol_render_ws* L, const float* v_img, const float* v_depth, const float* v_alpha,
                              int use_l1_sign, const float* l1_mask, int l1_mask_c, const float* v_img_scale,
                              float v_img_scale_mul, float* grad_records, float* v_mean, float* v_scale, float* v_quat, float* v_opacity,
                              float* v_colors, void* stream) {
  GOL_REQUIRE(workspace != nullptr && L != nullptr && grad_records != nullptr, "null workspace / layout / gradient records");
  GOL_REQUIRE(!use_l1_sign || L->l1_sign >= 0, "layout was computed without the fused L1");
  if (B == 0 || N == 0) return GOL_OK;
  void* ws = workspace;
  const float* g = grad_records;
  const bool use_depth = v_depth != nullptr;
  int rc = render_bwd_to_records(B, N, img_h, img_w, at<float>(ws, L->records), background, capacity, ws, L, v_img, v_depth,
                                 v_alpha, use_l1_sign, l1_mask, l1_mask_c, v_img_scale, v_img_scale_mul, grad_records,
                                 stream);
  if (rc != GOL_OK) return rc;
  return gol_project_bwd_records(B, N, means, scales, glob_scale, quats, viewmats, intrins, at<int32_t>(ws, L->radii),
                                 at<float>(ws, L->conics), at<float>(ws, L->comp), opacity, g, use_depth ? 1 : 0, v_mean,
                                 v_scale, v_quat, v_opacity, v_colors, stream);
}

extern "C" int gol_render_bwd_projected(int B, int N, const gol_shade_proj* proj, const float* background, int64_t capacity,
                                        void* workspace, const gol_render_ws* L, const float* v_img, const float* v_depth,
                                        const float* v_alpha, int use_l1_sign, const float* l1_mask, int l1_mask_c,
                                        const float* v_img_scale, float v_img_scale_mul, float* grad_records,
                                        void* stream) {
  GOL_REQUIRE(workspace != nullptr && L != nullptr && proj != nullptr && grad_records != nullptr,
              "null workspace / layout / projection / gradient records");
  GOL_REQUIRE(!use_l1_sign || L->l1_sign >= 0, "layout was computed without the fused L1");
  if (B == 0 || N == 0) return GOL_OK;
  return render_bwd_to_records(B, N, proj->img_h, proj->img_w, proj->records, background, capacity, workspace, L, v_img,
                               v_depth, v_alpha, use_l1_sign, l1_mask, l1_mask_c, v_img_scale, v_img_scale_mul,
                               grad_records, stream);
}
```

### goliath_amd/splat.py

```python
import ctypes
import math
import os

import torch

from . import _lib, views as _views
from ._lib import c_float, c_i64, c_int, fptr, ptr, stream_ptr

BLOCK = 16
GRAD_RECORD = 16
SPLAT_RECORD = 16

def _tiles(img_h, img_w, block=BLOCK):
    return ((img_w + block - 1) // block) * ((img_h + block - 1) // block)


class CapacityPlanner:

    def __init__(self):
        self.capacity = {}
        self.mode = os.environ.get("GOLIATH_CAPACITY_MODE", "adaptive")
        self.pending = []
        self.frozen = False
        self.frozen_log = []
        self.reruns = 0
        self.truncated = 0
        self.last_worst = {}
        self.force_block = set()
        self._pinned = {}

    def check_frozen(self):
        for n_isect, capacity in self.frozen_log:
            worst = int(n_isect.max()) if n_isect.numel() else 0
            if worst > capacity:
                raise _lib.GoliathHipError(f"a captured render_views call overflowed its intersection capacity "
                                           f"({worst} > {capacity}): re-capture with a larger capacity")

    def must_block(self, key):
        if self.mode == "verify" or os.environ.get("GOLIATH_STRICT_CAPACITY", "0") == "1":
            return True
        if self.mode == "async":
            return False
        seen, cap = self.last_worst.get(key), self.capacity.get(key)
        return key in self.force_block or seen is None or cap is None or seen * 1.5 > cap

    def passed(self, key):
        self.force_block.discard(key)

    def get(self, key):
        return self.capacity.get(key)

    def initial(self, N, T):
        return int(min(2**31 - 1, max(1 << 16, 16 * N + T)))

    def set(self, key, counts_max):
        want = int(min(2**31 - 1, max(1 << 16, int(counts_max * 2.0) + 4096)))
        self.capacity[key] = max(self.capacity.get(key, 0), want)
        return self.capacity[key]

    def observe(self, key, worst, capacity):
        self.last_worst[key] = worst
        if key not in self.capacity or worst * 1.5 > capacity:
            self.set(key, worst)

    def _take_pinned(self, B):
        free = self._pinned.setdefault(B, [])
        return free.pop() if free else torch.empty(B, dtype=torch.int32, pin_memory=True)

    def fetch(self, n_isect):
        B = n_isect.numel()
        host = self._take_pinned(B)
        host.copy_(n_isect, non_blocking=True)
        ev = torch.cuda.Event()
        ev.record()
        return host, ev

    def finish(self, host, ev):
        ev.synchronize()
        worst = int(host.max()) if host.numel() else 0
        self._pinned[host.numel()].append(host)
        return worst

    def note(self, key, n_isect, capacity):
        host, ev = self.fetch(n_isect)
        self.pending.append((ev, host, capacity, key))

    def poll(self, block=False):
        still, overflow = [], None
        for ev, host, capacity, key in self.pending:
            if block:
                ev.synchronize()
            if ev.query():
                worst = int(host.max()) if host.numel() else 0
                self._pinned[host.numel()].append(host)
                if worst > capacity:
                    self.last_worst[key] = worst
                    self.set(key, worst)
                    self.force_block.add(key)
                    overflow = (worst, capacity, key)
                else:
                    self.observe(key, worst, capacity)
            else:
                still.append((ev, host, capacity, key))
        self.pending = still
        if overflow is not None:
            worst, capacity, key = overflow
            msg = (f"a previous render_views call overflowed its intersection capacity ({worst} > {capacity}): its tile "
                   f"lists were truncated. Capacity was raised to {self.capacity[key]}")
            if self.mode == "async":
                raise _lib.GoliathHipError(msg + " -- re-run the step (GOLIATH_CAPACITY_MODE=verify repairs inside the "
                                                 "call instead).")
            import sys
            import warnings

            self.truncated += 1
            try:
                frame = sys._getframe(2)
            except ValueError:
                frame = sys._getframe(0)
            warnings.warn_explicit(msg + "; calls of this shape check their own counts before returning until one has passed "
                                         "(GOLIATH_CAPACITY_MODE=verify checks every call).", CapacityWarning,
                                   frame.f_code.co_filename, frame.f_lineno, module=frame.f_globals.get("__name__"), registry={})


class CapacityWarning(RuntimeWarning):
    """A render_views call was found, after the fact, to have rendered with truncated tile lists (adaptive mode)."""


PLANNER = CapacityPlanner()


class _Workspace:

    def __init__(self, B, N, T, capacity, device):
        self.capacity = capacity
        self.tile_count = torch.zeros(B, T, dtype=torch.int32, device=device)
        self.tile_bins = torch.empty(B, T, 2, dtype=torch.int32, device=device)
        self.keys = torch.empty(B, max(capacity, 1), dtype=torch.int64, device=device)
        self.sorted_ids = torch.empty(B, max(capacity, 1), dtype=torch.int32, device=device)
        self.n_isect = torch.empty(B, dtype=torch.int32, device=device)
        self.reach = torch.empty(B, max(N, 1), dtype=torch.int64, device=device)


_F32, _I32, _I64, _U8 = torch.float32, torch.int32, torch.int64, torch.uint8


def _p(x, dtype=_F32, name="tensor"):
    return ctypes.c_void_p(x) if x is None or isinstance(x, int) else ptr(x, dtype, name)


def _abi_bin_sort(*, B, N, xys, depths, radii, conics=None, opacities=None, img_h, img_w, capacity, tile_count, tile_bins,
                  isect_keys, sorted_ids, n_isect, reach_scratch=None):
    _lib.call("gol_bin_sort", c_int(B), c_int(N), _p(xys), _p(depths), _p(radii, _I32), _p(conics), _p(opacities),
              c_int(img_h), c_int(img_w), c_int(BLOCK), c_i64(capacity), _p(tile_count, _I32), _p(tile_bins, _I32),
              _p(isect_keys, _I64), _p(sorted_ids, _I32), _p(n_isect, _I32), _p(reach_scratch, _I64), stream_ptr())


def _abi_project_fwd(*, B, N, means3d, scales, glob_scale, quats, viewmats, intrins, img_h, img_w, clip_thresh, cov3d=None,
                     xys, depths, radii, conics, compensation, num_tiles_hit=None, opacities=None, opac_eff=None,
                     colors=None, records=None):
    _lib.call("gol_project_fwd", c_int(B), c_int(N), _p(means3d, name="means3d"), _p(scales, name="scales"),
              c_float(glob_scale), _p(quats, name="quats"), _p(viewmats, name="viewmat"), _p(intrins, name="intrins"),
              c_int(img_h), c_int(img_w), c_int(BLOCK), c_float(clip_thresh), _p(cov3d), _p(xys), _p(depths),
              _p(radii, _I32), _p(conics), _p(compensation), _p(num_tiles_hit, _I32), _p(opacities, name="opacity"),
              _p(opac_eff), _p(colors, name="colors"), _p(records), stream_ptr())


def _abi_project_bwd(*, B, N, means3d, scales, glob_scale, quats, viewmats, intrins, cov3d=None, radii, conics, compensation,
                     v_xy=None, v_depth=None, v_conic=None, v_compensation=None, opacities=None, v_opac_eff=None,
                     grad_stride=0, v_mean3d, v_scale, v_quat, v_opacity=None):
    _lib.call("gol_project_bwd", c_int(B), c_int(N), _p(means3d), _p(scales), c_float(glob_scale), _p(quats),
              _p(viewmats), _p(intrins), _p(cov3d), _p(radii, _I32), _p(conics), _p(compensation), _p(v_xy), _p(v_depth),
              _p(v_conic), _p(v_compensation), _p(opacities), _p(v_opac_eff), c_int(grad_stride), _p(v_mean3d),
              _p(v_scale), _p(v_quat), _p(v_opacity), stream_ptr())


def _abi_rasterize_fwd(*, B, N, img_h, img_w, planar, tile_bins, sorted_ids, capacity, records, with_extra, background,
                       out_img, out_extra=None, final_Ts, final_idx, out_alpha=None, out_extra_norm=None, norm_lo=0.0,
                       l1_target=None, l1_mask=None, l1_mask_c=0, l1_sign=None, l1_partial=None, l1_out=None,
                       l1_scale=1.0, pixels_per_lane=0):
    _lib.call("gol_rasterize_fwd", c_int(B), c_int(N), c_int(img_h), c_int(img_w), c_int(BLOCK), c_int(planar),
              _p(tile_bins, _I32), _p(sorted_ids, _I32), c_i64(capacity), _p(records), c_int(with_extra),
              _p(background), _p(out_img), _p(out_extra), _p(final_Ts), _p(final_idx, _I32), _p(out_alpha),
              _p(out_extra_norm), c_float(norm_lo), _p(l1_target), _p(l1_mask), c_int(l1_mask_c), _p(l1_sign, _U8),
              _p(l1_partial), _p(l1_out), c_float(l1_scale), c_int(pixels_per_lane), stream_ptr())


def _abi_rasterize_bwd(*, B, N, img_h, img_w, planar, tile_bins, sorted_ids, capacity, records, with_extra, background,
                       final_Ts, final_idx, v_out_img=None, v_out_extra=None, v_out_alpha=None, v_xy, v_conic, v_colors,
                       v_extra=None, v_opacity, grad_stride=0, v_sign=None, v_sign_mask=None, v_sign_mask_c=0,
                       v_img_scale=None, v_img_scale_mul=1.0, pixels_per_lane=0):
    _lib.call("gol_rasterize_bwd", c_int(B), c_int(N), c_int(img_h), c_int(img_w), c_int(BLOCK), c_int(planar),
              _p(tile_bins, _I32), _p(sorted_ids, _I32), c_i64(capacity), _p(records), c_int(with_extra), _p(background),
              _p(final_Ts), _p(final_idx, _I32), _p(v_out_img), _p(v_out_extra), _p(v_out_alpha), _p(v_xy), _p(v_conic),
              _p(v_colors), _p(v_extra), _p(v_opacity), c_int(grad_stride), _p(v_sign, _U8), _p(v_sign_mask),
              c_int(v_sign_mask_c), _p(v_img_scale), c_float(v_img_scale_mul), c_int(pixels_per_lane), stream_ptr())


def _abi_rasterize_nd_fwd(*, B, N, C, img_h, img_w, tile_bins, sorted_ids, capacity, records, colors, background, out_img,
                          final_Ts, final_idx, pixels_per_lane=0):
    _lib.call("gol_rasterize_nd_fwd", c_int(B), c_int(N), c_int(C), c_int(img_h), c_int(img_w), c_int(BLOCK),
              _p(tile_bins, _I32), _p(sorted_ids, _I32), c_i64(capacity), _p(records), _p(colors), _p(background),
              _p(out_img), _p(final_Ts), _p(final_idx, _I32), c_int(pixels_per_lane), stream_ptr())


def _abi_rasterize_nd_bwd(*, B, N, C, img_h, img_w, tile_bins, sorted_ids, capacity, records, colors, background, final_Ts,
                          final_idx, v_out_img, v_out_alpha=None, v_xy, v_conic, v_colors, v_opacity):
    _lib.call("gol_rasterize_nd_bwd", c_int(B), c_int(N), c_int(C), c_int(img_h), c_int(img_w), c_int(BLOCK),
              _p(tile_bins, _I32), _p(sorted_ids, _I32), c_i64(capacity), _p(records), _p(colors), _p(background),
              _p(final_Ts), _p(final_idx, _I32), _p(v_out_img), _p(v_out_alpha), _p(v_xy), _p(v_conic), _p(v_colors),
              _p(v_opacity), stream_ptr())


def _bin_sort(B, N, xys, depths, radii, img_h, img_w, ws, conics=None, opacities=None):
    _abi_bin_sort(B=B, N=N, xys=xys, depths=depths, radii=radii, conics=conics, opacities=opacities, img_h=img_h,
                  img_w=img_w, capacity=ws.capacity, tile_count=ws.tile_count, tile_bins=ws.tile_bins, isect_keys=ws.keys,
                  sorted_ids=ws.sorted_ids, n_isect=ws.n_isect, reach_scratch=ws.reach)


def _project_fwd(B, N, means, scales, glob_scale, quats, viewmats, intrins, img_h, img_w, clip,
                 opacities=None, colors=None):
    f = dict(dtype=torch.float32, device=means.device)
    records = torch.empty(B, N, SPLAT_RECORD, **f) if colors is not None else None
    cov3d, xys, conics = (torch.empty(B, N, k, **f) for k in (6, 2, 3))
    depths, comp = torch.empty(B, N, **f), torch.empty(B, N, **f)
    radii, nth = (torch.empty(B, N, dtype=torch.int32, device=means.device) for _ in range(2))
    opac_eff = torch.empty(B, N, **f) if opacities is not None else None
    _abi_project_fwd(B=B, N=N, means3d=means, scales=scales, glob_scale=glob_scale, quats=quats, viewmats=viewmats,
                     intrins=intrins, img_h=img_h, img_w=img_w, clip_thresh=clip, cov3d=cov3d, xys=xys, depths=depths,
                     radii=radii, conics=conics, compensation=comp, num_tiles_hit=nth, opacities=opacities,
                     opac_eff=opac_eff, colors=colors, records=records)
    out = (cov3d, xys, depths, radii, conics, comp, nth, opac_eff)
    return out + (records,) if colors is not None else out


def _pack_records(B, N, xys, conics, colors, extra, opacities):
    records = torch.empty(B, N, SPLAT_RECORD, dtype=torch.float32, device=xys.device)
    _lib.call("gol_splat_pack", c_int(B), c_int(N), fptr(xys), fptr(conics), fptr(colors), fptr(extra), fptr(opacities),
              fptr(records), stream_ptr())
    return records


def _f32c(t):
    return t.to(torch.float32).contiguous()


class _ProjectGaussians(torch.autograd.Function):
    @staticmethod
    def forward(ctx, means3d, scales, glob_scale, quats, viewmat, fx, fy, cx, cy, img_height, img_width,
                block_width, clip_thresh):
        if block_width != BLOCK:
            raise NotImplementedError("goliath_amd implements block_width=16 (the reference's value)")
        N = means3d.shape[0]
        dev = means3d.device
        means3d, scales, quats = _f32c(means3d), _f32c(scales), _f32c(quats)
        vm = _f32c(viewmat).reshape(-1)[:12].contiguous().view(1, 12)
        intr = torch.tensor([[fx, fy, cx, cy]], dtype=torch.float32).to(dev, non_blocking=True)
        with _lib.device_guard(dev):
            cov3d, xys, depths, radii, conics, comp, nth, _ = _project_fwd(
                1, N, means3d, scales, float(glob_scale), quats, vm, intr, img_height, img_width,
                float(clip_thresh))
        ctx.save_for_backward(means3d, scales, quats, vm, intr, cov3d[0], radii[0], conics[0], comp[0])
        ctx.glob_scale = float(glob_scale)
        ctx.set_materialize_grads(False)
        outs = (xys[0], depths[0], radii[0], conics[0], comp[0], nth[0], cov3d[0])
        ctx.mark_non_differentiable(outs[2], outs[5])
        return outs

    @staticmethod
    def backward(ctx, v_xys, v_depths, v_radii, v_conics, v_compensation, v_num_tiles_hit, v_cov3d):
        means3d, scales, quats, vm, intr, cov3d, radii, conics, comp = ctx.saved_tensors
        N = means3d.shape[0]
        v_mean = torch.empty_like(means3d)
        v_scale = torch.empty_like(scales)
        v_quat = torch.empty_like(quats)
        c = lambda t: None if t is None else _f32c(t)
        g_xy, g_depth, g_conic, g_comp = c(v_xys), c(v_depths), c(v_conics), c(v_compensation)
        with _lib.device_guard(means3d.device):
            _abi_project_bwd(B=1, N=N, means3d=means3d, scales=scales, glob_scale=ctx.glob_scale, quats=quats, viewmats=vm,
                             intrins=intr, cov3d=cov3d, radii=radii, conics=conics, compensation=comp, v_xy=g_xy,
                             v_depth=g_depth, v_conic=g_conic, v_compensation=g_comp, v_mean3d=v_mean, v_scale=v_scale,
                             v_quat=v_quat)
        return (v_mean, v_scale, None, v_quat) + (None,) * 9



def project_gaussians(means3d, scales, glob_scale, quats, viewmat, fx, fy, cx, cy, img_height, img_width,
                      block_width, clip_thresh=0.01):
    if means3d.dim() != 2 or means3d.shape[1] != 3:
        raise ValueError("means3d must have dimensions (N, 3)")
    return _ProjectGaussians.apply(means3d, scales, glob_scale, quats, viewmat, fx, fy, cx, cy, img_height,
                                   img_width, block_width, clip_thresh)


class _RasterizeGaussians(torch.autograd.Function):
    @staticmethod
    def forward(ctx, xys, depths, radii, conics, num_tiles_hit, colors, opacity, img_height, img_width,
                block_width, background, return_alpha):
        dev = xys.device
        N, C = xys.shape[0], colors.shape[-1]
        xys, depths, conics, colors = _f32c(xys), _f32c(depths), _f32c(conics), _f32c(colors)
        opacity = _f32c(opacity).reshape(-1)
        radii = radii.to(torch.int32).contiguous()
        background = _f32c(background)
        n_isect = int(num_tiles_hit.to(torch.int64).sum().item()) if N > 0 else 0
        ctx.n_isect = n_isect
        ctx.dims = (img_height, img_width)
        if n_isect < 1:
            out_img = torch.ones(img_height, img_width, C, device=dev) * background
            final_Ts = torch.zeros(img_height, img_width, device=dev)
            ctx.save_for_backward(xys, conics, colors, opacity, background)
        else:
            T = _tiles(img_height, img_width)
            ws = _Workspace(1, N, T, n_isect, dev)
            out_img = torch.empty(1, img_height, img_width, C, device=dev)
            final_Ts = torch.empty(1, img_height, img_width, device=dev)
            final_idx = torch.empty(1, img_height, img_width, dtype=torch.int32, device=dev)
            with _lib.device_guard(dev):
                _bin_sort(1, N, xys, depths, radii, img_height, img_width, ws, conics, opacity)
                if C == 3:
                    records = _pack_records(1, N, xys, conics, colors, None, opacity)
                    _abi_rasterize_fwd(B=1, N=N, img_h=img_height, img_w=img_width, planar=0, tile_bins=ws.tile_bins,
                                       sorted_ids=ws.sorted_ids, capacity=ws.capacity, records=records, with_extra=0,
                                       background=background, out_img=out_img, final_Ts=final_Ts, final_idx=final_idx)
                else:
                    records = _pack_records(1, N, xys, conics, None, None, opacity)
                    _abi_rasterize_nd_fwd(B=1, N=N, C=C, img_h=img_height, img_w=img_width, tile_bins=ws.tile_bins,
                                          sorted_ids=ws.sorted_ids, capacity=ws.capacity, records=records, colors=colors,
                                          background=background, out_img=out_img, final_Ts=final_Ts, final_idx=final_idx)
            ctx.ws = ws
            ctx.save_for_backward(xys, conics, colors, opacity, background, final_Ts, final_idx, records)
            out_img, final_Ts = out_img[0], final_Ts[0]
        if return_alpha:
            return out_img, 1 - final_Ts
        return out_img

    @staticmethod
    def backward(ctx, v_out_img, v_out_alpha=None):
        saved = ctx.saved_tensors
        xys, conics, colors, opacity, background = saved[:5]
        N = xys.shape[0]
        v_xy = torch.zeros_like(xys)
        v_conic = torch.zeros_like(conics)
        v_colors = torch.zeros_like(colors)
        v_opacity = torch.zeros(N, device=xys.device)
        if ctx.n_isect >= 1 and v_out_img is not None:
            final_Ts, final_idx, records = saved[5], saved[6], saved[7]
            H, W = ctx.dims
            ws = ctx.ws
            va = None if v_out_alpha is None else _f32c(v_out_alpha)
            vo = _f32c(v_out_img)
            with _lib.device_guard(xys.device):
                if colors.shape[-1] == 3:
                    _abi_rasterize_bwd(B=1, N=N, img_h=H, img_w=W, planar=0, tile_bins=ws.tile_bins,
                                       sorted_ids=ws.sorted_ids, capacity=ws.capacity, records=records, with_extra=0,
                                       background=background, final_Ts=final_Ts, final_idx=final_idx, v_out_img=vo,
                                       v_out_alpha=va, v_xy=v_xy, v_conic=v_conic, v_colors=v_colors, v_opacity=v_opacity)
                else:
                    _abi_rasterize_nd_bwd(B=1, N=N, C=colors.shape[-1], img_h=H, img_w=W, tile_bins=ws.tile_bins,
                                          sorted_ids=ws.sorted_ids, capacity=ws.capacity, records=records, colors=colors,
                                          background=background, final_Ts=final_Ts, final_idx=final_idx, v_out_img=vo,
                                          v_out_alpha=va, v_xy=v_xy, v_conic=v_conic, v_colors=v_colors,
                                          v_opacity=v_opacity)
        return (v_xy, None, None, v_conic, None, v_colors, v_opacity[:, None]) + (None,) * 5


def rasterize_gaussians(xys, depths, radii, conics, num_tiles_hit, colors, opacity, img_height, img_width,
                        block_width, background=None, return_alpha=False):
    assert block_width > 1 and block_width <= 16, "block_width must be between 2 and 16"
    if block_width != BLOCK:
        raise NotImplementedError("goliath_amd implements block_width=16 (the reference's value)")
    if colors.dtype == torch.uint8:
        colors = colors.float() / 255
    if xys.ndimension() != 2 or xys.size(1) != 2:
        raise ValueError("xys must have dimensions (N, 2)")
    if colors.ndimension() != 2:
        raise ValueError("colors must have dimensions (N, D)")
    if background is not None:
        assert background.shape[0] == colors.shape[-1], "incorrect shape of background color tensor"
    else:
        background = torch.ones(colors.shape[-1], dtype=torch.float32, device=colors.device)
    if opacity.ndimension() != 2 or opacity.shape[1] != 1:
        opacity = opacity.reshape(-1, 1)
    return _RasterizeGaussians.apply(xys.contiguous(), depths.contiguous(), radii.contiguous(),
                                     conics.contiguous(), num_tiles_hit.contiguous(), colors.contiguous(),
                                     opacity.contiguous(), img_height, img_width, block_width,
                                     background.contiguous(), return_alpha)


class RenderLayout(ctypes.Structure):
    _fields_ = [(n, ctypes.c_int64) for n in (
        "cov3d", "xys", "depths", "radii", "conics", "comp", "nth", "opac_eff", "records", "tile_count", "tile_bins",
        "keys", "sorted_ids", "n_isect", "final_T", "final_idx", "l1_sign", "total")]


_LAYOUTS = {}


def _layout(B, N, img_h, img_w, capacity, with_l1, projected=False):
    key = (B, N, img_h, img_w, capacity, with_l1, projected)
    L = _LAYOUTS.get(key)
    if L is None:
        L = RenderLayout()
        _lib.call("gol_render_layout_projected" if projected else "gol_render_layout", c_int(B), c_int(N), c_int(img_h),
                  c_int(img_w), c_i64(capacity), c_int(with_l1), ctypes.byref(L))
        if len(_LAYOUTS) > 256:
            _LAYOUTS.clear()
        _LAYOUTS[key] = L
    return L


def _ws_view(ws, off, dtype, shape):
    return ws[off:off + math.prod(shape) * dtype.itemsize].view(dtype).view(shape)


def _render_fwd_staged(B, N, src, attrs, background, with_depth, norm_lo, cap, ws, L, out_img, out_depth, alpha, depth_norm,
                       l1_target, l1_mask, l1_mask_c, l1_partial, l1_out, l1_scale):
    a = ws.data_ptr()
    if attrs is not None:
        means, scales, quats, opacity, colors = attrs
        _abi_project_fwd(B=B, N=N, means3d=means, scales=scales, glob_scale=src.glob_scale, quats=quats,
                         viewmats=src.viewmats, intrins=src.intrins, img_h=src.img_h, img_w=src.img_w,
                         clip_thresh=src.clip_thresh, xys=src.xys, depths=src.depths, radii=src.radii, conics=src.conics,
                         compensation=src.comp, opacities=opacity, opac_eff=src.opac_eff, colors=colors,
                         records=src.records)
    _abi_bin_sort(B=B, N=N, xys=src.xys, depths=src.depths, radii=src.radii, conics=src.conics, opacities=src.opac_eff,
                  img_h=src.img_h, img_w=src.img_w, capacity=cap, tile_count=a + L.tile_count, tile_bins=a + L.tile_bins,
                  isect_keys=a + L.keys, sorted_ids=a + L.sorted_ids, n_isect=a + L.n_isect)
    _abi_rasterize_fwd(B=B, N=N, img_h=src.img_h, img_w=src.img_w, planar=1, tile_bins=a + L.tile_bins,
                       sorted_ids=a + L.sorted_ids, capacity=cap, records=src.records, with_extra=int(with_depth),
                       background=background, out_img=out_img, out_extra=out_depth, final_Ts=a + L.final_T,
                       final_idx=a + L.final_idx, out_alpha=alpha, out_extra_norm=depth_norm, norm_lo=norm_lo,
                       l1_target=l1_target, l1_mask=l1_mask, l1_mask_c=l1_mask_c,
                       l1_sign=a + L.l1_sign if l1_target is not None else None, l1_partial=l1_partial, l1_out=l1_out,
                       l1_scale=l1_scale)


def _render_bwd_staged(B, N, src, attrs, grads, background, cap, ws, L, v_img, v_depth, v_alpha, use_l1, l1_mask, v_scale,
                       v_scale_mul, rec):
    a = ws.data_ptr()
    field = lambda k: rec.data_ptr() + 4 * k
    use_depth = v_depth is not None
    rec.zero_()
    _abi_rasterize_bwd(B=B, N=N, img_h=src.img_h, img_w=src.img_w, planar=1, tile_bins=a + L.tile_bins,
                       sorted_ids=a + L.sorted_ids, capacity=cap, records=src.records, with_extra=int(use_depth),
                       background=background, final_Ts=a + L.final_T, final_idx=a + L.final_idx, v_out_img=v_img,
                       v_out_extra=v_depth, v_out_alpha=v_alpha, v_xy=field(4), v_conic=field(6), v_colors=field(0),
                       v_extra=field(9) if use_depth else None, v_opacity=field(3), grad_stride=GRAD_RECORD,
                       v_sign=a + L.l1_sign if use_l1 else None, v_sign_mask=l1_mask,
                       v_sign_mask_c=0 if l1_mask is None else l1_mask.shape[1], v_img_scale=v_scale,
                       v_img_scale_mul=v_scale_mul)
    if attrs is not None:
        means, scales, quats, opacity = attrs
        v_mean, v_scale_g, v_quat, v_opacity = grads
        _abi_project_bwd(B=B, N=N, means3d=means, scales=scales, glob_scale=src.glob_scale, quats=quats,
                         viewmats=src.viewmats, intrins=src.intrins, radii=src.radii, conics=src.conics,
                         compensation=src.comp, v_xy=field(4), v_depth=field(9) if use_depth else None, v_conic=field(6),
                         opacities=opacity, v_opac_eff=field(3), grad_stride=GRAD_RECORD, v_mean3d=v_mean,
                         v_scale=v_scale_g, v_quat=v_quat, v_opacity=v_opacity)


class _RenderViews(torch.autograd.Function):

    @staticmethod
    def forward(ctx, means, scales, quats, opacity, colors, viewmats, intrins, background, img_h, img_w,
                glob_scale, clip_thresh, with_depth, capacity, depth_norm_lo, plan_key, l1_target, l1_mask,
                raw_depth, records, pack, view_set, res):
        projected = records is not None
        B, N = (records if projected else means).shape[:2]
        dev = (records if projected else means).device
        pj = _views.proj_struct(view_set, records, pack) if projected else None
        attrs = None if projected else (means, scales, quats, opacity, colors)
        T = _tiles(img_h, img_w)
        with_l1 = 1 if l1_target is not None else 0
        f = dict(dtype=torch.float32, device=dev)
        out_img = torch.empty(B, 3, img_h, img_w, **f)
        out_depth = torch.empty(B, img_h, img_w, **f) if with_depth and raw_depth else None
        alpha = torch.empty(B, img_h, img_w, **f)
        depth_norm = torch.empty(B, img_h, img_w, **f) if with_depth else None
        l1_partial = torch.empty(B, T, **f) if with_l1 else None
        l1_out = torch.empty(1, **f) if with_l1 else None
        l1_inv_n = 1.0 / max(B * 3 * img_h * img_w, 1)
        l1_mask_c = 0 if l1_mask is None else l1_mask.shape[1]

        def run(cap):
            L = _layout(B, N, img_h, img_w, cap, with_l1, projected)
            ws = torch.empty(max(L.total, 1), dtype=torch.uint8, device=dev)
            a = ws.data_ptr()
            src = pj if projected else _views.ShadeProj(
                fptr(viewmats).value, fptr(intrins).value, img_h, img_w, glob_scale, clip_thresh, a + L.xys, a + L.depths,
                a + L.radii, a + L.conics, a + L.comp, a + L.opac_eff, a + L.records)
            if _lib.TIMING is not None:
                _render_fwd_staged(B, N, src, attrs, background, with_depth, depth_norm_lo, cap, ws, L, out_img, out_depth,
                                   alpha, depth_norm, l1_target, l1_mask, l1_mask_c, l1_partial, l1_out, l1_inv_n)
            else:
                entry = (("gol_render_fwd_projected", c_int(B), c_int(N), ctypes.byref(pj)) if projected else
                         ("gol_render_fwd", c_int(B), c_int(N), c_int(img_h), c_int(img_w), c_float(glob_scale),
                          c_float(clip_thresh), fptr(means), fptr(scales), fptr(quats), fptr(opacity), fptr(colors),
                          fptr(viewmats), fptr(intrins)))
                _lib.call(*entry, fptr(background), c_int(1 if with_depth else 0), c_float(depth_norm_lo), c_i64(cap),
                          ctypes.c_void_p(ws.data_ptr()), ctypes.byref(L), fptr(out_img), fptr(out_depth), fptr(alpha),
                          fptr(depth_norm), fptr(l1_target), fptr(l1_mask), c_int(l1_mask_c), fptr(l1_partial),
                          fptr(l1_out), c_float(l1_inv_n), stream_ptr())
            n_isect = _ws_view(ws, L.n_isect, torch.int32, (B,))
            pending = PLANNER.fetch(n_isect) if plan_key is not None and B > 0 else None
            return ws, L, src, n_isect, pending

        with _lib.device_guard(dev):
            ws, L, src, n_isect, pending = run(capacity)
            if pending is not None:
                worst = PLANNER.finish(*pending)
                if worst > capacity:
                    capacity = PLANNER.set(plan_key, worst)
                    PLANNER.last_worst[plan_key] = worst
                    PLANNER.reruns += 1
                    ws, L, src, n_isect, pending = run(capacity)
                    PLANNER.finish(*pending)
                else:
                    PLANNER.observe(plan_key, worst, capacity)
                PLANNER.passed(plan_key)
        res.bind((B, N, img_h, img_w, T), ws, L, capacity, src, pack if projected else ws, records if projected else ws)
        ctx.L, ctx.capacity, ctx.src = L, capacity, src
        ctx.cfg = (img_h, img_w, glob_scale, with_depth, depth_norm_lo, with_l1)
        ctx.l1_inv_n = l1_inv_n
        l1 = l1_out.reshape(()) if with_l1 else None
        ctx.view_set = view_set
        ctx.save_for_backward(means, scales, quats, opacity, viewmats, intrins, background, ws, l1_mask, records, pack)
        ctx.mark_non_differentiable(ws, n_isect)
        ctx.set_materialize_grads(False)
        return out_img, alpha, out_depth, depth_norm, l1, ws, n_isect

    @staticmethod
    def backward(ctx, v_img, v_alpha, v_depth, v_depth_norm, v_l1, *_non_differentiable):
        means, scales, quats, opacity, viewmats, intrins, background, ws, l1_mask, records, pack = ctx.saved_tensors
        img_h, img_w, glob_scale, with_depth, depth_norm_lo, with_l1 = ctx.cfg
        projected = records is not None
        B, N = (records if projected else means).shape[:2]
        dev = ws.device
        L = ctx.L
        if v_depth_norm is not None:
            final_Ts = _ws_view(ws, L.final_T, torch.float32, (B, img_h, img_w))
            g = v_depth_norm / (1.0 - final_Ts).clamp(depth_norm_lo, 1.0)
            v_depth = g if v_depth is None else v_depth + g
        if not with_l1:
            v_l1 = None
        if v_img is None and v_alpha is None and v_depth is None and v_l1 is None:
            return (None,) * 23
        v_scale = None
        if v_l1 is not None:
            v_scale = v_l1.to(torch.float32).reshape(1).contiguous()
        if v_img is None and v_l1 is None:
            v_img = torch.zeros(B, 3, img_h, img_w, device=dev)
        use_depth = with_depth and v_depth is not None
        v_img_c = None if v_img is None else _f32c(v_img)
        v_depth_c = _f32c(v_depth) if use_depth else None
        v_alpha_c = None if v_alpha is None else _f32c(v_alpha)
        rec = torch.empty(B, N, GRAD_RECORD, device=dev)
        use_mask = l1_mask if v_l1 is not None else None
        attrs = None if projected else (means, scales, quats, opacity)
        grads = None if projected else tuple(torch.empty_like(t) for t in attrs)
        with _lib.device_guard(dev):
            if _lib.TIMING is not None:
                _render_bwd_staged(B, N, ctx.src, attrs, grads, background, ctx.capacity, ws, L, v_img_c, v_depth_c,
                                   v_alpha_c, v_l1 is not None, use_mask, v_scale, ctx.l1_inv_n, rec)
                v_color = None if projected else rec[..., :3]
            else:
                shared = (fptr(background), c_i64(ctx.capacity), ctypes.c_void_p(ws.data_ptr()), ctypes.byref(L),
                          fptr(v_img_c), fptr(v_depth_c), fptr(v_alpha_c), c_int(1 if v_l1 is not None else 0),
                          fptr(use_mask), c_int(0 if use_mask is None else use_mask.shape[1]), fptr(v_scale),
                          c_float(ctx.l1_inv_n), fptr(rec))
                if projected:
                    _lib.call("gol_render_bwd_projected", c_int(B), c_int(N), ctypes.byref(ctx.src), *shared, stream_ptr())
                else:
                    v_color = torch.empty(B, N, 3, device=dev)
                    _lib.call("gol_render_bwd", c_int(B), c_int(N), c_int(img_h), c_int(img_w), c_float(glob_scale),
                              fptr(means), fptr(scales), fptr(quats), fptr(opacity), fptr(viewmats), fptr(intrins), *shared,
                              *(fptr(g) for g in grads), fptr(v_color), stream_ptr())
        if projected:
            return (None,) * 19 + (rec, None, None, None)
        return grads + (v_color,) + (None,) * 18


_BLACK = {}


class _LazyRender(dict):

    def bind(self, dims, ws, L, cap, src, arrays, records):
        self._dims, self._ws, self._L, self._cap, self._src, self._arrays, self._records = dims, ws, L, cap, src, arrays, records

    def __missing__(self, key):
        B, N, H, W, T = self._dims
        ws, L = self._ws, self._L
        if key == "radii":
            buf = self._arrays.view(-1).view(torch.uint8)
            v = _ws_view(buf, (self._src.radii or 0) - buf.data_ptr(), torch.int32, (B, N))
        elif key == "final_T":
            v = _ws_view(ws, L.final_T, torch.float32, (B, 1, H, W))
        elif key == "final_idx":
            v = _ws_view(ws, L.final_idx, torch.int32, (B, H, W))
        elif key == "sorted_ids":
            v = _ws_view(ws, L.sorted_ids, torch.int32, (B, max(self._cap, 1)))
        elif key == "tile_bins":
            v = _ws_view(ws, L.tile_bins, torch.int32, (B, T, 2))
        else:
            raise KeyError(key)
        self[key] = v
        return v


def raster_pair_counts(res):
    B, N, H, W, T = res._dims
    ws, L = res._ws, res._L
    a = ws.data_ptr()
    counts = torch.empty(B, 2, dtype=torch.int64, device=ws.device)
    with _lib.device_guard(ws.device):
        _lib.call("gol_raster_count_pairs", c_int(B), c_int(N), c_int(H), c_int(W), _p(a + L.tile_bins),
                  _p(a + L.sorted_ids), c_i64(res._cap), _p(res._src.records), _p(a + L.final_idx), _p(counts, _I64),
                  stream_ptr())
    return counts


def render_views(means, scales, quats, opacity, colors, viewmats, intrins, img_h, img_w,
                 background=None, glob_scale=1.0, clip_thresh=0.1, with_depth=True, capacity=None, depth_norm_lo=0.05,
                 l1_target=None, l1_mask=None, raw_depth=True, projected=None, extra_colors=None):
    if extra_colors is not None:
        BN = tuple((projected.records if projected is not None else means).shape[:2])
        if extra_colors.dim() != 3 or tuple(extra_colors.shape[:2]) != BN or extra_colors.shape[2] < 1:
            raise ValueError("extra_colors must be [B,N,Ce]")
        ins = (means, scales, quats, opacity, colors, extra_colors) + (() if projected is None else (projected.records,))
        if torch.is_grad_enabled() and any(t is not None and t.requires_grad for t in ins):
            raise _lib.GoliathHipError("render_views(extra_colors=...) is forward-only: call it under torch.no_grad() or "
                                       "with detached inputs")
        if not extra_colors.is_cuda:
            raise _lib.GoliathHipError("render_views needs CUDA(HIP) tensors; there is no CPU path")
    if projected is not None:
        B, N = projected.records.shape[:2]
        dev = projected.records.device
        if (projected.views.height, projected.views.width) != (img_h, img_w):
            raise ValueError("projected for another image size")
        means = scales = quats = opacity = colors = viewmats = intrins = None
        glob_scale, clip_thresh = projected.views.glob_scale, projected.views.clip_thresh
    else:
        B, N = means.shape[:2]
        dev = means.device
        if not means.is_cuda:
            raise _lib.GoliathHipError("render_views needs CUDA(HIP) tensors; there is no CPU path")
        means, scales, quats, colors = _f32c(means), _f32c(scales), _f32c(quats), _f32c(colors)
        opacity = _f32c(opacity).reshape(B, N)
        viewmats = _f32c(viewmats).reshape(B, viewmats[0].numel() if B else 12)[:, :12].contiguous()
        intrins = _f32c(intrins).reshape(B, 4)
    if background is None:
        background = _BLACK.get(dev)
        if background is None:
            background = _BLACK[dev] = torch.zeros(3, device=dev)
    background = _f32c(background)
    T = _tiles(img_h, img_w)
    key = (B, N, img_h, img_w, dev.index)
    plan_key, deferred = None, False
    if capacity is None:
        planned = PLANNER.get(key)
        if PLANNER.frozen:
            if planned is None:
                raise _lib.GoliathHipError("render_views inside a graph capture needs a calibrated capacity: run the "
                                           "same shapes once eagerly first")
        else:
            if PLANNER.pending:
                PLANNER.poll()
                planned = PLANNER.get(key)
            if planned is None or PLANNER.must_block(key):
                plan_key = key
            else:
                deferred = True
        capacity = planned if planned is not None else PLANNER.initial(N, T)
    if l1_target is not None:
        l1_target = _f32c(l1_target.detach())
        if tuple(l1_target.shape) != (B, 3, img_h, img_w):
            raise ValueError("l1_target must be [B,3,H,W]")
        if l1_mask is not None:
            l1_mask = _f32c(l1_mask.detach())
            if l1_mask.dim() != 4 or l1_mask.shape[0] != B or l1_mask.shape[1] not in (1, 3):
                raise ValueError("l1_mask must be [B,1,H,W] or [B,3,H,W]")
    else:
        l1_mask = None
    res = _LazyRender()
    img, alpha, depth, depth_norm, l1, _, n_isect = _RenderViews.apply(
        means, scales, quats, opacity, colors, viewmats, intrins, background, img_h, img_w, float(glob_scale),
        float(clip_thresh), bool(with_depth), int(capacity), float(depth_norm_lo), plan_key, l1_target, l1_mask,
        bool(raw_depth), None if projected is None else projected.records, None if projected is None else projected.pack,
        None if projected is None else projected.views, res)
    if PLANNER.frozen:
        PLANNER.frozen_log.append((n_isect, res._cap))
    elif deferred and B > 0:
        PLANNER.note(key, n_isect, res._cap)
    res["render"], res["alpha"], res["n_isect"] = img, alpha[:, None], n_isect
    if with_depth:
        if depth is not None:
            res["depth"] = depth[:, None]
        res["depth_norm"] = depth_norm[:, None]
    if l1 is not None:
        res["l1_loss"] = l1
    if extra_colors is not None:
        res["extra"] = _raster_extra(res, extra_colors)
    return res


def _raster_extra(res, extra_colors):
    B, N, H, W, _ = res._dims
    ws, L = res._ws, res._L
    extra_colors = _f32c(extra_colors.detach())
    Ce = extra_colors.shape[2]
    dev = ws.device
    out = torch.empty(B, H, W, Ce, dtype=torch.float32, device=dev)
    if B == 0 or N == 0:
        return out.zero_().permute(0, 3, 1, 2).contiguous()
    final_Ts = torch.empty(B, H, W, dtype=torch.float32, device=dev)
    final_idx = torch.empty(B, H, W, dtype=torch.int32, device=dev)
    a = ws.data_ptr()
    with _lib.device_guard(dev):
        _abi_rasterize_nd_fwd(B=B, N=N, C=Ce, img_h=H, img_w=W, tile_bins=a + L.tile_bins, sorted_ids=a + L.sorted_ids,
                              capacity=res._cap, records=res._src.records, colors=extra_colors,
                              background=torch.zeros(Ce, dtype=torch.float32, device=dev), out_img=out, final_Ts=final_Ts,
                              final_idx=final_idx)
    return out.permute(0, 3, 1, 2).contiguous()
```

### include/goliath_hip.h

```cpp
#ifndef GOLIATH_HIP_H
#define GOLIATH_HIP_H

#include <stddef.h>
#include <stdint.h>

#ifdef __cplusplus
extern "C" {
#endif

typedef enum {
  GOL_OK = 0,
  GOL_ERR_INVALID_ARG = -1,
  GOL_ERR_LAUNCH = -2,
  GOL_ERR_UNSUPPORTED = -3
} gol_status;

const char* gol_version(void);
const char* gol_last_error(void);
int gol_selftest_wave_sum4(const float* in256, float* out128, void* stream);

int gol_sg_eval_fwd(int N, int D, int L, const float* lobe_dirs, const float* lobe_sigmas,
                    const float* light_values, const float* light_pts, const float* prim_pts,
                    const int32_t* n_lights, float* integral, int w_type, void* stream);
int gol_sg_eval_bwd(int N, int D, int L, const float* lobe_dirs, const float* lobe_sigmas,
                    const float* light_values, const float* light_pts, const float* prim_pts,
                    const int32_t* n_lights, const float* grad_integral, float* grad_dirs,
                    float* grad_sigmas, float* grad_light_values, int w_type, void* stream);

int gol_project_fwd(int B, int N, const float* means3d, const float* scales, float glob_scale,
                    const float* quats, const float* viewmats, const float* intrins, int img_h,
                    int img_w, int block, float clip_thresh, float* cov3d, float* xys,
                    float* depths, int32_t* radii, float* conics, float* compensation,
                    int32_t* num_tiles_hit, const float* opacities, float* opac_eff, const float* colors,
                    float* records, void* stream);
int gol_project_bwd(int B, int N, const float* means3d, const float* scales, float glob_scale,
                    const float* quats, const float* viewmats, const float* intrins,
                    const float* cov3d, const int32_t* radii, const float* conics,
                    const float* compensation, const float* v_xy, const float* v_depth,
                    const float* v_conic, const float* v_compensation, const float* opacities,
                    const float* v_opac_eff, int grad_stride, float* v_mean3d, float* v_scale, float* v_quat,
                    float* v_opacity, void* stream);
int gol_project_bwd_records(int B, int N, const float* means3d, const float* scales, float glob_scale,
                            const float* quats, const float* viewmats, const float* intrins, const int32_t* radii,
                            const float* conics, const float* compensation, const float* opacities,
                            const float* grad_records, int with_depth, float* v_mean3d, float* v_scale, float* v_quat,
                            float* v_opacity, float* v_colors, void* stream);

int gol_bin_sort(int B, int N, const float* xys, const float* depths, const int32_t* radii,
                 const float* conics, const float* opacities, int img_h, int img_w, int block,
                 int64_t capacity, int32_t* tile_count, int32_t* tile_bins, uint64_t* isect_keys,
                 int32_t* sorted_ids, int32_t* n_isect, uint64_t* reach_scratch, void* stream);

#define GOL_GRAD_RECORD 16
#define GOL_SPLAT_RECORD 16
int gol_splat_pack(int B, int N, const float* xys, const float* conics, const float* colors, const float* extra,
                   const float* opacities, float* records, void* stream);
int gol_rasterize_fwd(int B, int N, int img_h, int img_w, int block, int planar, const int32_t* tile_bins,
                      const int32_t* sorted_ids, int64_t capacity, const float* records, int with_extra,
                      const float* background, float* out_img,
                      float* out_extra, float* final_Ts, int32_t* final_idx, float* out_alpha,
                      float* out_extra_norm, float norm_lo, const float* l1_target, const float* l1_mask, int l1_mask_c,
                      uint8_t* l1_sign, float* l1_partial, float* l1_out, float l1_scale, int pixels_per_lane,
                      void* stream);
int gol_rasterize_bwd(int B, int N, int img_h, int img_w, int block, int planar, const int32_t* tile_bins,
                      const int32_t* sorted_ids, int64_t capacity, const float* records, int with_extra,
                      const float* background, const float* final_Ts,
                      const int32_t* final_idx, const float* v_out_img, const float* v_out_extra,
                      const float* v_out_alpha, float* v_xy, float* v_conic, float* v_colors,
                      float* v_extra, float* v_opacity, int grad_stride, const uint8_t* v_sign, const float* v_sign_mask,
                      int v_sign_mask_c, const float* v_img_scale, float v_img_scale_mul, int pixels_per_lane,
                      void* stream);
int gol_raster_count_pairs(int B, int N, int img_h, int img_w, const int32_t* tile_bins, const int32_t* sorted_ids,
                           int64_t capacity, const float* records, const int32_t* final_idx, uint64_t* counts, void* stream);
int gol_raster_plan(int B, int* fwd_pixels_per_lane);

int gol_rasterize_nd_fwd(int B, int N, int C, int img_h, int img_w, int block, const int32_t* tile_bins,
                         const int32_t* sorted_ids, int64_t capacity, const float* records, const float* colors,
                         const float* background, float* out_img, float* final_Ts, int32_t* final_idx,
                         int pixels_per_lane, void* stream);
int gol_rasterize_nd_bwd(int B, int N, int C, int img_h, int img_w, int block, const int32_t* tile_bins,
                         const int32_t* sorted_ids, int64_t capacity, const float* records, const float* colors,
                         const float* background, const float* final_Ts, const int32_t* final_idx,
                         const float* v_out_img, const float* v_out_alpha, float* v_xy, float* v_conic,
                         float* v_colors, float* v_opacity, void* stream);

typedef struct gol_render_ws {
  int64_t cov3d, xys, depths, radii, conics, comp, nth, opac_eff, records, tile_count, tile_bins, keys, sorted_ids,
      n_isect, final_T, final_idx, l1_sign, total;
} gol_render_ws;
int gol_render_layout(int B, int N, int img_h, int img_w, int64_t capacity, int with_l1, gol_render_ws* layout);
int gol_render_fwd(int B, int N, int img_h, int img_w, float glob_scale, float clip_thresh, const float* means,
                   const float* scales, const float* quats, const float* opacity, const float* colors,
                   const float* viewmats, const float* intrins, const float* background, int with_depth, float norm_lo,
                   int64_t capacity, void* workspace, const gol_render_ws* layout, float* out_img, float* out_depth,
                   float* out_alpha, float* out_depth_norm, const float* l1_target, const float* l1_mask, int l1_mask_c,
                   float* l1_partial, float* l1_out, float l1_scale, void* stream);
int gol_render_bwd(int B, int N, int img_h, int img_w, float glob_scale, const float* means, const float* scales,
                   const float* quats, const float* opacity, const float* viewmats, const float* intrins,
                   const float* background, int64_t capacity, void* workspace, const gol_render_ws* layout,
                   const float* v_img, const float* v_depth, const float* v_alpha, int use_l1_sign, const float* l1_mask,
                   int l1_mask_c, const float* v_img_scale, float v_img_scale_mul, float* grad_records, float* v_mean,
                   float* v_scale, float* v_quat, float* v_opacity, float* v_colors, void* stream);

#define GOL_MAX_MIPS 8
typedef struct {
  int32_t B, N;
  int32_t n_color_coef;
  int32_t n_mono_coef;
  const float* f_vnocond;
  const float* f_vcond;
  const float* postex;
  const float* tn;
  const float* albedo;
  const float* light_sh;
  const float* light_sh_rand;
  const float* campos;
  int32_t L;
  const float* light_intensity;
  const float* light_pos;
  const int32_t* n_lights;
  int32_t n_mips;
  const float* mips[GOL_MAX_MIPS];
  int32_t mip_h[GOL_MAX_MIPS], mip_w[GOL_MAX_MIPS];
  const float* lightrot;
  const float* mips_packed[GOL_MAX_MIPS];
  float primscale_min, primscale_max;
  int32_t mips_shared;
  float mips_scale;
  const float* mips_scale_dev;
} gol_shade_in;

typedef struct {
  float* color;
  float* opacity;
  float* primpos;
  float* primqvec;
  float* primscale;
  float* primscale_preclip;
  float* sigma;
  float* spec_vis;
  float* spec_nml;
  float* spec_dnml;
  float* diff_color;
  float* spec_color;
  float* primnmlbase;
  float* color_rand;
  float* diff_sum;
  float* env_saved;
} gol_shade_out;

typedef struct {
  const float *color, *opacity, *primpos, *primqvec, *primscale, *primscale_preclip, *sigma, *spec_vis,
      *spec_nml, *spec_dnml, *diff_color, *spec_color, *primnmlbase, *color_rand;
} gol_shade_out_grad;

typedef struct {
  float* f_vnocond;
  float* f_vcond;
  float* postex;
  float* tn;
  float* albedo_per_view;
  float* albedo;
} gol_shade_in_grad;

int gol_envmap_pack(int B, int h, int w, const float* src, float* dst, void* stream);
int gol_shade_fwd(const gol_shade_in* in, const gol_shade_out* out, void* stream);
int gol_shade_bwd(const gol_shade_in* in, const gol_shade_out* saved, const gol_shade_out_grad* g,
                  const gol_shade_in_grad* gin, void* stream);

typedef struct {
  const float* viewmats;
  const float* intrins;
  int32_t img_h, img_w;
  float glob_scale, clip_thresh;
  float* xys;
  float* depths;
  int32_t* radii;
  float* conics;
  float* comp;
  float* opac_eff;
  float* records;
} gol_shade_proj;
int gol_shade_project_fwd(const gol_shade_in* in, const gol_shade_out* out, const gol_shade_proj* proj, void* stream);
int gol_render_layout_projected(int B, int N, int img_h, int img_w, int64_t capacity, int with_l1, gol_render_ws* layout);
int gol_render_fwd_projected(int B, int N, const gol_shade_proj* proj, const float* background, int with_depth,
                             float norm_lo, int64_t capacity, void* workspace, const gol_render_ws* layout,
                             float* out_img, float* out_depth, float* out_alpha, float* out_depth_norm,
                             const float* l1_target, const float* l1_mask, int l1_mask_c, float* l1_partial, float* l1_out,
                             float l1_scale, void* stream);
int gol_render_bwd_projected(int B, int N, const gol_shade_proj* proj, const float* background, int64_t capacity,
                             void* workspace, const gol_render_ws* layout, const float* v_img, const float* v_depth,
                             const float* v_alpha, int use_l1_sign, const float* l1_mask, int l1_mask_c,
                             const float* v_img_scale, float v_img_scale_mul, float* grad_records, void* stream);
int gol_shade_project_bwd(const gol_shade_in* in, const gol_shade_out* saved, const gol_shade_out_grad* g,
                          const gol_shade_proj* proj, const float* grad_records, int with_depth,
                          const gol_shade_in_grad* gin, void* stream);

int gol_raydirs_fwd(int N, int H, int W, const float* viewpos, const float* viewrot, const float* focal,
                    const float* princpt, const float* pixelcoords , float volradius,
                    float* raypos, float* raydir, float* tminmax, void* stream);
int gol_mvp_aabb(int N, int K, const float* primpos, const float* primrot, const float* primscale,
                 float* nodeaabb, void* stream);
int gol_mvp_march_fwd(int N, int H, int W, int K, const float* raypos, const float* raydir, float stepsize,
                      const float* tminmax, const float* nodeaabb, const float* primpos,
                      const float* primrot, const float* primscale, const float* tplate, int TD, int TH,
                      int TW, float fadescale, float fadeexp, float* rayrgba, float* raysat, float* shadow,
                      void* stream);
int gol_mvp_march_bwd(int N, int H, int W, int K, const float* raypos, const float* raydir, float stepsize,
                      const float* tminmax, const float* nodeaabb, const float* primpos,
                      const float* primrot, const float* primscale, const float* tplate, int TD, int TH,
                      int TW, float fadescale, float fadeexp, const float* raysat, const float* grad_rayrgba,
                      float* grad_primpos, float* grad_primrot, float* grad_primscale, float* grad_tplate,
                      void* stream);

int gol_mvp_march_warp_fwd(int N, int H, int W, int K, const float* raypos, const float* raydir, float stepsize,
                           const float* tminmax, const float* nodeaabb, const float* primpos,
                           const float* primrot, const float* primscale, const float* tplate, int TD, int TH,
                           int TW, const float* warp, int WD, int WH, int WW, float fadescale, float fadeexp,
                           float* rayrgba, float* raysat, float* shadow, void* stream);
int gol_mvp_march_warp_bwd(int N, int H, int W, int K, const float* raypos, const float* raydir, float stepsize,
                           const float* tminmax, const float* nodeaabb, const float* primpos,
                           const float* primrot, const float* primscale, const float* tplate, int TD, int TH,
                           int TW, const float* warp, int WD, int WH, int WW, float fadescale, float fadeexp,
                           const float* raysat, const float* grad_rayrgba, float* grad_primpos, float* grad_primrot,
                           float* grad_primscale, float* grad_tplate, float* grad_warp, void* stream);

int gol_mvp_shadow_march(int N, int group, int H, int W, int K, const float* raypos, const float* raydir,
                         float stepsize, const float* tminmax, const float* nodeaabb, const float* primpos,
                         const float* primrot, const float* primscale, const float* tplate, int alpha_only,
                         int TD, int TH, int TW, float fadescale, float fadeexp, float* rayrgba, float* shadow,
                         void* stream);

#define GOL_UV_MAX_POW 4
typedef struct {
  int32_t B, L, HW, n_pow;
  float pow[GOL_UV_MAX_POW];
  float fresnel;
  const float *p_uv, *nml, *cam_pos, *light_pos, *light_intensity, *shadow_map, *roughness, *tex_mean;
} gol_uvlight_in;
int gol_uvlight_phong_fwd(const gol_uvlight_in* in, float* diff, float* spec, void* stream);
int gol_uvlight_phong_bwd(const gol_uvlight_in* in, const float* u_diff, const float* u_spec, float* g_p_uv,
                          float* g_nml, void* stream);
int gol_uvlight_ggx_fwd(const gol_uvlight_in* in, float* feat, float* rgb, void* stream);
int gol_uvlight_ggx_bwd(const gol_uvlight_in* in, const float* u_feat, const float* u_rgb, float* g_p_uv,
                        float* g_nml, float* g_roughness, float* g_tex, void* stream);

int gol_l1_blocks(int HW);
int gol_l1_fwd(int B, int C, int HW, int mask_c, const float* pred, const float* target, const float* mask,
               float* partial, void* stream);
int gol_l1_bwd(int B, int C, int HW, int mask_c, const float* pred, const float* target, const float* mask,
               const float* g_loss, float* g_pred, void* stream);

int gol_tail_conv_fwd(int B, int Ci, int h, int w, int CH, int E, int nd, int wB, const float* x, const float* weff,
                      const float* lc, const float* bias, float* out, void* stream);
int gol_tail_conv_bwd(int B, int Ci, int h, int w, int CH, int E, int nd, int wB, const float* x, const float* weff_t,
                      const float* lc, const float* g_out, float* g_x, float* g_weff, float* g_bias, float* w_scratch,
                      void* stream);
long long gol_tail_conv_bwd_scratch_floats(int B, int h, int w, int CH);

int gol_trunk_conv_fwd(int B, int Ci, int Co, int h, int w, float leak, const float* x, const float* w_eff,
                       const float* bias, float* y, void* stream);
long long gol_trunk_conv_bwd_scratch_floats(int B, int Ci, int Co, int h, int w);
int gol_trunk_conv_bwd(int B, int Ci, int Co, int h, int w, float leak, const float* x, const float* w_eff_t,
                       const float* y, const float* g_y, float* g_x, float* g_w, float* g_bias, float* scratch,
                       void* stream);

int gol_ssim_blocks(int H, int W);
int gol_ssim_fwd(int B, int C, int H, int W, int mask_c, const float* img1, const float* img2, const float* mask,
                 float* partial, float* dmap, void* stream);
int gol_ssim_bwd(int B, int C, int H, int W, const float* img1, const float* img2, const float* dmap,
                 const float* g_scale, float* g_img2, void* stream);

int gol_shadow_pcf(int B, int L, int H, int W, int dh, int dw, const float* depth, const float* Rt, float fx, float fy,
                   float cx, float cy, const float* postex, const float* nml, float exp_scale, float* out,
                   void* stream);

int64_t gol_imgtail_partial_floats(int B, int H, int W);
int gol_imgtail_fwd(int B, int H, int W, const float* rgb, const float* alpha, const float* bg,
                    const float* bg_scale, const float* cal_M, const float* cal_b, const float* blur_w,
                    float* out, void* stream);
int gol_imgtail_bwd(int B, int H, int W, const float* rgb, const float* alpha, const float* bg,
                    const float* bg_scale, const float* cal_M, const float* cal_b, const float* blur_w,
                    const float* g_out, float* g_rgb, float* partials, void* stream);

int64_t gol_mesh_raster_workspace_bytes(int B, int F);
int gol_mesh_raster(int B, int V, int F, int H, int W, const float* v_pix, const int32_t* vi, int32_t* index_img,
                    float* depth_img, float* bary_img, void* workspace, void* stream);

int gol_mesh_render_fwd(int B, int F, int Vt, int C, int H, int W, int Ht, int Wt, const float* vt, const int32_t* vti,
                        const float* tex, const int32_t* index_img, const float* bary_img, float* vt_img, float* render,
                        float* mask, void* stream);
int gol_mesh_render_bwd(int B, int V, int F, int Vt, int C, int H, int W, int Ht, int Wt, const float* v_pix,
                        const int32_t* vi, const float* vt, const int32_t* vti, const float* tex, const int32_t* index_img,
                        const float* bary_img, const float* g_render, const float* g_vt_img, const float* g_bary_img,
                        const float* g_depth_img, float* g_tex, float* g_v_pix, void* stream);
int gol_mesh_render_edge_bwd(int B, int V, int F, int C, int H, int W, const float* v_pix, const int32_t* vi,
                             const int32_t* index_img, const float* depth_img, const float* render,
                             const float* g_render, float* g_v_pix, int32_t* edge_stats, void* stream);

int gol_vert_normals_fwd(int B, int V, int F, const float* verts, const int32_t* vi, const int32_t* vf_start,
                         const int32_t* vf_slot, float eps, float* vn, void* stream);
int gol_vert_normals_bwd(int B, int V, int F, const float* verts, const int32_t* vi, const int32_t* vf_start,
                         const int32_t* vf_slot, float eps, const float* g_vn, float* g_s, float* g_verts, void* stream);
int gol_values_to_uv_fwd(int B, int V, int C, int S, int T, const float* values, const int32_t* texel_rec,
                         const int32_t* triples, float* out, void* stream);
int gol_values_to_uv_bwd(int B, int V, int C, int S, int T, int I, const int32_t* texel_rec, const int32_t* item_start,
                         const int32_t* texel_of, const int32_t* vt_start, const int32_t* vt_slot, const float* g_out,
                         float* item_sums, float* g_values, void* stream);
int gol_uvgeom_fwd(int B, int V, int F, int S, int T, const float* verts, const int32_t* vi, const int32_t* vf_start,
                   const int32_t* vf_slot, const int32_t* texel_rec, const int32_t* triples, float vn_eps, float norm_eps,
                   float* vn, float* postex, float* tn, void* stream);
int gol_uvgeom_bwd(int B, int V, int F, int S, int T, int I, const float* verts, const int32_t* vi,
                   const int32_t* vf_start, const int32_t* vf_slot, const int32_t* texel_rec, const int32_t* triples,
                   const int32_t* item_start, const int32_t* item_tid, const int32_t* texel_of, const int32_t* vt_start,
                   const int32_t* vt_slot, float vn_eps, float norm_eps, const float* vn, const float* g_postex,
                   const float* g_tn, float* item_sums, float* g_s, float* g_verts, void* stream);

int gol_lbs_skeleton_fwd(int B, int J, int NP, int NS, int L, const float* poses, const float* scales, int scales_stride,
                         const float* transform_t, const float* transform_offsets, const float* joint_offset,
                         const float* joint_rotation, const double* bind_inv, const int32_t* parents,
                         const int32_t* level_start, const int32_t* level_joints, float* states, float* mats,
                         void* stream);
int gol_lbs_skeleton_bwd(int B, int J, int NP, int NS, int L, const float* poses, const float* scales, int scales_stride,
                         const float* transform, const float* transform_t, const float* transform_offsets,
                         const float* joint_offset, const float* joint_rotation, const double* bind_inv,
                         const int32_t* parents, const int32_t* level_start, const int32_t* level_joints,
                         const int32_t* child_start, const int32_t* child_slot, const float* g_states,
                         const float* g_mats, float* g_poses, float* g_scales, void* stream);
int gol_lbs_skin_fwd(int B, int V, int J, int K, const float* mats, const float* verts, int verts_batched,
                     const float* template_verts, const float* global_scaling, const int32_t* skin_indices,
                     const float* skin_weights, float* out, void* stream);
int gol_lbs_skin_bwd(int B, int V, int J, int K, int E, int I, const float* mats, const float* verts, int verts_batched,
                     const float* template_verts, const float* global_scaling, const int32_t* skin_indices,
                     const float* skin_weights, const int32_t* item_start, const int32_t* jv_slot,
                     const int32_t* ji_start, const float* g_out, double* item_sums, float* g_verts, float* g_mats,
                     void* stream);

#define GOL_OPTIM_GROUP_DOUBLES 8
#define GOL_OPTIM_SCRUB 1
#define GOL_OPTIM_CLIP 2
#define GOL_OPTIM_WRITE_BACK 4
int gol_optim_chunk_elems(void);
int gol_optim_grad_stats(int n_chunks, int n_seg, const int32_t* chunk_seg, const int64_t* chunk_off, const int64_t* seg_g,
                         const int64_t* seg_numel, double* partial, void* stream);
int gol_optim_finalize(int n_chunks, const double* partial, double max_norm, double* stats, int64_t* nonfinite,
                       void* stream);
int gol_optim_adam_step(int n_chunks, int n_seg, int n_groups, const int32_t* chunk_seg, const int64_t* chunk_off,
                        const int64_t* seg_p, const int64_t* seg_g, const int64_t* seg_m, const int64_t* seg_v,
                        const int64_t* seg_step, const int64_t* seg_numel, const int32_t* seg_group, const double* groups,
                        const double* stats, float* seg_coef, int flags, void* stream);

typedef enum {
  GOL_REGLOSS_BOUND = 0,
  GOL_REGLOSS_NEG_SQ = 1,
  GOL_REGLOSS_SQ = 2,
  GOL_REGLOSS_ABS = 3,
  GOL_REGLOSS_ALPHAPRIOR = 4
} gol_regloss_kind;
int gol_regloss_chunk_elems(void);
int gol_regloss_fwd(int kind, int64_t n, float p0, float p1, const float* x, double* partial, void* stream);
int gol_regloss_bwd(int kind, int64_t n, float p0, float p1, const float* x, const float* g_scale, float* g_x,
                    void* stream);
int gol_backlit_fwd(int64_t m, int c, const float* color, const float* cosw, double* partial, void* stream);
int gol_backlit_bwd(int64_t m, int c, const float* color, const float* cosw, const float* g_scale, float* g_color,
                    void* stream);

typedef enum {
  GOL_IMGLOSS_ABS = 0,
  GOL_IMGLOSS_SQ = 1,
  GOL_IMGLOSS_EXPW = 2
} gol_imgloss_kind;
int gol_imgloss_chunk_elems(void);
int gol_imgloss_fwd(int kind, int B, int C, int HW, int mask_c, const float* pred, const float* target, const float* mask,
                    const uint8_t* veto, double* partial, void* stream);
int gol_imgloss_finalize(int64_t n_chunks, int64_t n, const double* partial, float* loss, double* sum, void* stream);
int gol_imgloss_bwd(int kind, int B, int C, int HW, int mask_c, const float* pred, const float* target, const float* mask,
                    const uint8_t* veto, const float* g_scale, float* g_pred, void* stream);
int gol_depth_disc_mask(int B, int H, int W, int pool, float threshold, const float* depth, uint8_t* out, void* stream);
int gol_mask_erode(int B, int H, int W, int ks, int x_is_u8, const void* x, float* out, void* stream);

int gol_envbg_blur_taps(double* taps );
int64_t gol_envbg_scratch_floats(int B, int H, int W);
int gol_envbg_image(int B, int H, int W, int He, int We, const float* envbg, const float* K, const float* R,
                    double focal_scale, int blur, float* scratch, float* bg, void* stream);
int gol_envbg_compose(int B, int H, int W, int He, int We, const float* render, const float* alpha, const float* bg,
                      const float* envbg, const float* R, int ball, float* out, void* stream);

int gol_sh_norm_constants(int deg, double* out );
int gol_sh_basis_fwd(int M, int deg, const float* dirs, float* coeffs, void* stream);
int gol_light_sh_fwd(int B, int L, int deg, const float* light_pos, const float* light_intensity, int intensity_channels,
                     const float* head_pose, float* headrel_light_pos, float* light_sh, void* stream);

int64_t gol_envspin_scratch_floats(int B, int H, int W);
int gol_envspin_frame(int B, int H, int W, const float* image, const float* rot, const int32_t* tap_y_start,
                      const double* tap_y_w, int ky, const int32_t* tap_x_start, const double* tap_x_w, int kx,
                      float perc90, double env_scale, float* scratch, float* envbg, float* envmap, float* light_intensity,
                      float* norm_scale, float* mip_scale, void* stream);

int gol_mvp_template_fwd(int B, int TD, int TH, int TW, int ny, int nx, const float* rgb, const float* alpha,
                         const int32_t* slot, const int32_t* live, int Kout, int act, float rgb_scale, float rgb_shift,
                         float* out, float* out_full, void* stream);
int gol_mvp_template_bwd(int B, int TD, int TH, int TW, int ny, int nx, const float* rgb, const float* alpha,
                         const int32_t* slot, const int32_t* live, int Kout, int act, float rgb_scale, float rgb_shift,
                         const float* g_out, const float* g_out_full, float* g_rgb, float* g_alpha, void* stream);
int gol_mvp_primtransf_fwd(int B, int K, const float* posbase, const float* rotbase, const float* delta_pos,
                           const float* delta_rvec, const float* delta_scale, float prim_scale, float* primpos,
                           float* primrot, float* primscale, void* stream);
int gol_mvp_primtransf_bwd(int B, int K, const float* rotbase, const float* delta_rvec, float prim_scale,
                           const float* g_primpos, const float* g_primrot, const float* g_primscale, float* g_delta_pos,
                           float* g_delta_rvec, float* g_delta_scale, void* stream);

int64_t gol_envprefilter_scratch_floats(int B, int He, int We);
int gol_envprefilter_sg(int B, int H, int W, int He, int We, int S, double sigma, const float* v, const float* env_tex,
                        const float* xi, int64_t seed, int64_t sample_offset, float* scratch, float* out, void* stream);

#ifdef __cplusplus
}
#endif
#endif
```

Measured before the change: 3002 views/s.

## Cache per-entry wave masks from forward and simplify backward alpha-gradient recurrence

```diff
diff --git a/goliath_amd/csrc/gol_raster.h b/goliath_amd/csrc/gol_raster.h
--- a/goliath_amd/csrc/gol_raster.h
+++ b/goliath_amd/csrc/gol_raster.h
@@ -93,6 +93,13 @@
   s.mask = wave_mask<PPL>(q0.x, q0.y, cn.x, cn.y, cn.z, q2.z, q2.w, q3.x, q3.y, tile_x0, tile_y0);
   return s;
 }
+__device__ __forceinline__ Staged stage_entry_masked(const float* __restrict__ records, size_t g, int mask) {
+  const float4* R = reinterpret_cast<const float4*>(records + g * GOL_SPLAT_RECORD);
+  const float4 q0 = R[0], q1 = R[1], q2 = R[2];
+  Staged s;
+  s.a = q0; s.b = q1; s.c = make_float2(q2.x, q2.y); s.mask = mask;
+  return s;
+}
 
 template <typename V, int P>
 __device__ __forceinline__ bool any_live(const V& live) {
@@ -187,11 +194,11 @@
 
 template <int PPL>
 __device__ __forceinline__ void bwd_moments(const fvec<PPL>& e, const fvec<PPL>& w, const fvec<PPL>& T_cur,
-                                            const fvec<PPL>& ra, const fvec<PPL>& fac, const fvec<PPL>& tail,
-                                            const bool (&v)[PPL], const fvec<PPL>& dy, fvec<PPL>& qsum, fvec<PPL>& gop,
-                                            fvec<PPL>& gy, fvec<PPL>& gyy) {
-  const fvec<PPL> v_alpha = T_cur * w + ra * (tail - qsum);
-  qsum += fac * w;
+                                            const fvec<PPL>& alpha, const bool (&v)[PPL], const fvec<PPL>& dy,
+                                            fvec<PPL>& R, fvec<PPL>& gop, fvec<PPL>& gy, fvec<PPL>& gyy) {
+  const fvec<PPL> d = w - R;
+  const fvec<PPL> v_alpha = T_cur * d;
+  R += alpha * d;
   gop = e * v_alpha;
 #pragma unroll
   for (int q = 0; q < PPL; ++q) gop[q] = v[q] ? gop[q] : 0.f;
diff --git a/goliath_amd/csrc/raster.hip b/goliath_amd/csrc/raster.hip
--- a/goliath_amd/csrc/raster.hip
+++ b/goliath_amd/csrc/raster.hip
@@ -14,7 +14,8 @@
     float* __restrict__ out_extra, float* __restrict__ final_Ts, int32_t* __restrict__ final_idx,
     float* __restrict__ out_alpha, float* __restrict__ out_extra_norm, float norm_lo,
     const float* __restrict__ l1_target, const float* __restrict__ l1_mask, int l1_mask_c,
-    uint8_t* __restrict__ l1_sign, float* __restrict__ l1_partial, int n_views, int bg_group, int bg_vec16) {
+    uint8_t* __restrict__ l1_sign, float* __restrict__ l1_partial, int n_views, int bg_group, int bg_vec16,
+    uint8_t* __restrict__ stage_mask) {
   typedef typename Pix<PPL>::fv fv;
   typedef typename Pix<PPL>::iv iv;
   constexpr int NW = Pix<PPL>::kWaves, NT = 64 * NW;
@@ -161,6 +162,7 @@
 
   const int32_t* ids = sorted_ids + (size_t)view * capacity;
   const size_t goff = (size_t)view * N;
+  uint8_t* __restrict__ o_mask = (PPL == 2 && stage_mask) ? stage_mask + (size_t)view * capacity : nullptr;
 
   fv T_cur = 1.f;
   iv cur_idx = 0;
@@ -175,6 +177,7 @@
       if (idx < range.y) {
         const Staged st = stage_entry<PPL>(records, goff + (size_t)ids[idx], (float)(tc.tx * 16), (float)(tc.ty * 16));
         s_a[k] = st.a; s_b[k] = st.b; s_c[k] = st.c; s_mask[k] = st.mask;
+        if (PPL == 2 && o_mask) *gol_at(o_mask, (unsigned)idx) = (uint8_t)st.mask;
       } else {
         s_mask[k] = 0;
       }
@@ -323,7 +326,7 @@
     const float* __restrict__ v_out_alpha, float* __restrict__ v_xy, float* __restrict__ v_conic,
     float* __restrict__ v_colors, float* __restrict__ v_extra, float* __restrict__ v_opacity,
     const uint8_t* __restrict__ v_sign, const float* __restrict__ v_sign_mask, int v_sign_mask_c,
-    const float* __restrict__ v_img_scale, float v_img_scale_mul, int n_views) {
+    const float* __restrict__ v_img_scale, float v_img_scale_mul, int n_views, const uint8_t* __restrict__ stage_mask) {
   typedef typename Pix<PPL>::fv fv;
   typedef typename Pix<PPL>::iv iv;
   constexpr int NW = Pix<PPL>::kWaves, NT = 64 * NW;
@@ -387,8 +390,7 @@
       if (v_out_alpha) voa[q] = v_out_alpha[p];
     }
   }
-  const fv tail = T_final * (voa - (background[0] * vo0 + background[1] * vo1 + background[2] * vo2));
-  fv qsum = 0.f;
+  fv R = (background[0] * vo0 + background[1] * vo1 + background[2] * vo2) - voa;
 
   const int wmax = wave_last_entry<PPL>(bin_final);
   if (lane == 0) s_wmax[wave] = wmax;
@@ -405,24 +407,30 @@
     const int e = bmax - bb2 * kBatchB - tid;
     return (tid < kBatchB && e >= range.x) ? ids[e] : 0;
   };
-  int gid_next = entry_id(0);
+  const uint8_t* __restrict__ i_mask = stage_mask ? stage_mask + (size_t)view * capacity : nullptr;
+  auto entry_mask = [&](int bb2) {
+    const int e = bmax - bb2 * kBatchB - tid;
+    return (i_mask && tid < kBatchB && e >= range.x) ? (int)i_mask[e] : 0;
+  };
+  int gid_next = entry_id(0), mask_next = entry_mask(0);
   unsigned rec_bytes = GOL_GRAD_RECORD * sizeof(float);
   if (PACKED) asm volatile("" : "+s"(rec_bytes));
   for (int bb = 0; bb < n_batches; ++bb) {
     __syncthreads();
     const int batch_end = bmax - bb * kBatchB;
     const int batch_size = min(kBatchB, batch_end + 1 - range.x);
-    const int gid = gid_next;
+    const int gid = gid_next, mask = mask_next;
     if (tid < kBatchB) {
       if (tid < batch_size) {
-        const Staged st = stage_entry<PPL>(records, goff + (size_t)gid, (float)(tc.tx * 16), (float)(tc.ty * 16));
+        const Staged st = i_mask ? stage_entry_masked(records, goff + (size_t)gid, mask)
+                                 : stage_entry<PPL>(records, goff + (size_t)gid, (float)(tc.tx * 16), (float)(tc.ty * 16));
         s_e[tid].a = st.a; s_e[tid].b = st.b; s_e[tid].c = st.c; s_mask[tid] = st.mask;
         s_id[tid] = gid;
       } else {
         s_mask[tid] = 0;
       }
     }
-    if (bb + 1 < n_batches) gid_next = entry_id(bb + 1);
+    if (bb + 1 < n_batches) { gid_next = entry_id(bb + 1); mask_next = entry_mask(bb + 1); }
     (&s_touched[0][0])[tid] = 0;
     __syncthreads();
 
@@ -447,7 +455,7 @@
       fv w = b4.z * vo0 + b4.w * vo1 + c2.x * vo2;
       if (EXTRA) w += c2.y * vo3;
       fv gop, gy, gyy;
-      bwd_moments<PPL>(vis, w, T_cur, ra, fac, tail, v, dy, qsum, gop, gy, gyy);
+      bwd_moments<PPL>(vis, w, T_cur, alpha, v, dy, R, gop, gy, gyy);
       float g0s, g1s, g2s, g3 = 0.f;
       if (PPL == 2) {
         g0s = __builtin_fmaf(fac[0], vo0[0], fac[PPL - 1] * vo0[PPL - 1]);
@@ -609,6 +617,11 @@
                    colors ? colors[3 * e + 2] : 0.f, extra ? extra[e] : 0.f);
 }
 
+inline bool stage_mask_on() {
+  const char* e = getenv("GOL_RASTER_STAGE_MASK");
+  return !(e && e[0] == '0' && e[1] == 0);
+}
+
 }
 
 extern "C" int gol_raster_plan(int B, int* fwd_pixels_per_lane) {
@@ -654,7 +667,7 @@
                                  float* out_extra, float* final_Ts, int32_t* final_idx, float* out_alpha,
                                  float* out_extra_norm, float norm_lo, const float* l1_target, const float* l1_mask,
                                  int l1_mask_c, uint8_t* l1_sign, float* l1_partial, float* l1_out, float l1_scale,
-                                 int pixels_per_lane, void* stream) {
+                                 uint8_t* stage_mask, int pixels_per_lane, void* stream) {
   GOL_RASTER_CHECK_DIMS(12, "image too large (32-bit byte offsets inside a view)");
   if (B == 0) return GOL_OK;
   GOL_REQUIRE(tile_bins && background && out_img && final_Ts && final_idx, "null pointer");
@@ -691,7 +704,7 @@
       raster_fwd_kernel<EX, LZ, PPL><<<grid, 64 * Pix<PPL>::kWaves, 0, s>>>(
           N, img_h, img_w, planar, tiles_x, tiles_y, bins, sorted_ids, capacity, records, background, out_img, out_extra,
           final_Ts, final_idx, out_alpha, EX ? out_extra_norm : nullptr, norm_lo, l1_target, l1_mask, l1_mask_c, l1_sign,
-          l1_partial, B, bg_group, bg_vec16);
+          l1_partial, B, bg_group, bg_vec16, stage_mask_on() ? stage_mask : nullptr);
     });
   };
   const bool ex = out_extra || out_extra_norm;
@@ -711,7 +724,8 @@
                                  const float* v_out_alpha, float* v_xy, float* v_conic, float* v_colors,
                                  float* v_extra, float* v_opacity, int grad_stride, const uint8_t* v_sign,
                                  const float* v_sign_mask, int v_sign_mask_c, const float* v_img_scale,
-                                 float v_img_scale_mul, int pixels_per_lane, void* stream) {
+                                 float v_img_scale_mul, const uint8_t* stage_mask, int stage_mask_ppl, int pixels_per_lane,
+                                 void* stream) {
   GOL_RASTER_CHECK_DIMS(0, "");
   if (B == 0 || N == 0 || capacity == 0) return GOL_OK;
   GOL_REQUIRE(tile_bins && sorted_ids && background && final_Ts && final_idx, "null pointer");
@@ -732,7 +746,9 @@
   const int2* bins = reinterpret_cast<const int2*>(tile_bins);
   hipStream_t s = (hipStream_t)stream;
   GOL_REQUIRE(pixels_per_lane >= 0 && pixels_per_lane <= 2, "pixels_per_lane: 0 (2), 1 or 2");
+  GOL_REQUIRE(stage_mask_ppl >= 0 && stage_mask_ppl <= 2, "stage_mask_ppl: the forward's pixels_per_lane (1 or 2), 0 = no masks");
   const int ppl = pixels_per_lane ? pixels_per_lane : 2;
+  const uint8_t* masks = (stage_mask && stage_mask_ppl == 2 && ppl == 2 && stage_mask_on()) ? stage_mask : nullptr;
   const bool ex = with_extra && (v_out_extra || v_extra);
   auto launch = [&](auto ex_c, auto packed_c) {
     with_ppl(ppl, [&](auto ppl_c) {
@@ -741,7 +757,7 @@
       raster_bwd_kernel<EX, PK, PPL><<<grid, 64 * Pix<PPL>::kWaves, 0, s>>>(
           N, img_h, img_w, planar, tiles_x, tiles_y, bins, sorted_ids, capacity, records, background, final_Ts, final_idx,
           v_out_img, EX ? v_out_extra : nullptr, v_out_alpha, v_xy, v_conic, v_colors, EX ? v_extra : nullptr, v_opacity,
-          v_sign, v_sign_mask, v_sign_mask_c, v_img_scale, v_img_scale_mul, B);
+          v_sign, v_sign_mask, v_sign_mask_c, v_img_scale, v_img_scale_mul, B, masks);
     });
   };
   if (ex && packed) launch(kYes, kYes);
diff --git a/goliath_amd/csrc/raster_nd.hip b/goliath_amd/csrc/raster_nd.hip
--- a/goliath_amd/csrc/raster_nd.hip
+++ b/goliath_amd/csrc/raster_nd.hip
@@ -190,9 +190,8 @@
   fv bgdot = 0.f;
 #pragma unroll
   for (int c = 0; c < CK; ++c) bgdot += ((c < nc) ? background[c0 + c] : 0.f) * vo[c];
-  const fv tail = T_final * (voa - bgdot);
   fv T_cur = T_final;
-  fv qsum = 0.f;
+  fv R = bgdot - voa;
 
   float* acc_lane = &s_acc[wave][0][lane >> 4];
   const int n_batches = (bmax - range.x + kBatchNdB) / kBatchNdB;
@@ -237,7 +236,7 @@
 #pragma unroll
       for (int c = 0; c < CK; ++c) w += col[c] * vo[c];
       fv gop, gy, gyy;
-      bwd_moments<PPL>(vis, w, T_cur, ra, fac, tail, v, dy, qsum, gop, gy, gyy);
+      bwd_moments<PPL>(vis, w, T_cur, alpha, v, dy, R, gop, gy, gyy);
       float s[kRow];
 #pragma unroll
       for (int c = 0; c < CK; ++c) {
diff --git a/goliath_amd/csrc/render.hip b/goliath_amd/csrc/render.hip
--- a/goliath_amd/csrc/render.hip
+++ b/goliath_amd/csrc/render.hip
@@ -27,6 +27,7 @@
   L->tile_bins = take((int64_t)B * T * 2 * 4);
   L->keys = take((int64_t)B * cap * 8);
   L->sorted_ids = take((int64_t)B * cap * 4);
+  L->stage_mask = take((int64_t)B * cap);
   L->n_isect = take((int64_t)B * 4);
   L->final_T = take((int64_t)B * P * 4);
   L->final_idx = take((int64_t)B * P * 4);
@@ -58,8 +59,8 @@
                            capacity, records, with_depth ? 1 : 0, background, out_img,
                            with_depth ? out_depth : nullptr, at<float>(ws, L->final_T), at<int32_t>(ws, L->final_idx),
                            out_alpha, with_depth ? out_depth_norm : nullptr, norm_lo, l1_target, l1_mask, l1_mask_c,
-                           l1_target ? at<uint8_t>(ws, L->l1_sign) : nullptr, l1_partial, l1_out, l1_scale, 0,
-                           stream);
+                           l1_target ? at<uint8_t>(ws, L->l1_sign) : nullptr, l1_partial, l1_out, l1_scale,
+                           at<uint8_t>(ws, L->stage_mask), 0, stream);
 }
 
 static int render_bwd_to_records(int B, int N, int img_h, int img_w, const float* records, const float* background,
@@ -74,12 +75,15 @@
   }
   float* g = grad_records;
   const bool use_depth = v_depth != nullptr;
+  int fwd_ppl = 0;
+  gol_raster_plan(B, &fwd_ppl);
   return gol_rasterize_bwd(B, N, img_h, img_w, 16, 1, at<int32_t>(ws, L->tile_bins), at<int32_t>(ws, L->sorted_ids),
                            capacity, records, use_depth ? 1 : 0, background,
                            at<float>(ws, L->final_T), at<int32_t>(ws, L->final_idx), v_img, v_depth, v_alpha, g + 4, g + 6,
                            g, use_depth ? g + 9 : nullptr, g + 3, GOL_GRAD_RECORD,
                            use_l1_sign ? at<uint8_t>(ws, L->l1_sign) : nullptr, use_l1_sign ? l1_mask : nullptr,
-                           use_l1_sign ? l1_mask_c : 0, v_img_scale, v_img_scale_mul, 0, stream);
+                           use_l1_sign ? l1_mask_c : 0, v_img_scale, v_img_scale_mul, at<uint8_t>(ws, L->stage_mask),
+                           fwd_ppl, 0, stream);
 }
 
 extern "C" int gol_render_fwd(int B, int N, int img_h, int img_w, float glob_scale, float clip_thresh, const float* means,
diff --git a/goliath_amd/splat.py b/goliath_amd/splat.py
--- a/goliath_amd/splat.py
+++ b/goliath_amd/splat.py
@@ -178,23 +178,24 @@
 def _abi_rasterize_fwd(*, B, N, img_h, img_w, planar, tile_bins, sorted_ids, capacity, records, with_extra, background,
                        out_img, out_extra=None, final_Ts, final_idx, out_alpha=None, out_extra_norm=None, norm_lo=0.0,
                        l1_target=None, l1_mask=None, l1_mask_c=0, l1_sign=None, l1_partial=None, l1_out=None,
-                       l1_scale=1.0, pixels_per_lane=0):
+                       l1_scale=1.0, stage_mask=None, pixels_per_lane=0):
     _lib.call("gol_rasterize_fwd", c_int(B), c_int(N), c_int(img_h), c_int(img_w), c_int(BLOCK), c_int(planar),
               _p(tile_bins, _I32), _p(sorted_ids, _I32), c_i64(capacity), _p(records), c_int(with_extra),
               _p(background), _p(out_img), _p(out_extra), _p(final_Ts), _p(final_idx, _I32), _p(out_alpha),
               _p(out_extra_norm), c_float(norm_lo), _p(l1_target), _p(l1_mask), c_int(l1_mask_c), _p(l1_sign, _U8),
-              _p(l1_partial), _p(l1_out), c_float(l1_scale), c_int(pixels_per_lane), stream_ptr())
+              _p(l1_partial), _p(l1_out), c_float(l1_scale), _p(stage_mask, _U8), c_int(pixels_per_lane), stream_ptr())
 
 
 def _abi_rasterize_bwd(*, B, N, img_h, img_w, planar, tile_bins, sorted_ids, capacity, records, with_extra, background,
                        final_Ts, final_idx, v_out_img=None, v_out_extra=None, v_out_alpha=None, v_xy, v_conic, v_colors,
                        v_extra=None, v_opacity, grad_stride=0, v_sign=None, v_sign_mask=None, v_sign_mask_c=0,
-                       v_img_scale=None, v_img_scale_mul=1.0, pixels_per_lane=0):
+                       v_img_scale=None, v_img_scale_mul=1.0, stage_mask=None, stage_mask_ppl=0, pixels_per_lane=0):
     _lib.call("gol_rasterize_bwd", c_int(B), c_int(N), c_int(img_h), c_int(img_w), c_int(BLOCK), c_int(planar),
               _p(tile_bins, _I32), _p(sorted_ids, _I32), c_i64(capacity), _p(records), c_int(with_extra), _p(background),
               _p(final_Ts), _p(final_idx, _I32), _p(v_out_img), _p(v_out_extra), _p(v_out_alpha), _p(v_xy), _p(v_conic),
               _p(v_colors), _p(v_extra), _p(v_opacity), c_int(grad_stride), _p(v_sign, _U8), _p(v_sign_mask),
-              c_int(v_sign_mask_c), _p(v_img_scale), c_float(v_img_scale_mul), c_int(pixels_per_lane), stream_ptr())
+              c_int(v_sign_mask_c), _p(v_img_scale), c_float(v_img_scale_mul), _p(stage_mask, _U8), c_int(stage_mask_ppl),
+              c_int(pixels_per_lane), stream_ptr())
 
 
 def _abi_rasterize_nd_fwd(*, B, N, C, img_h, img_w, tile_bins, sorted_ids, capacity, records, colors, background, out_img,
@@ -391,7 +392,7 @@
 class RenderLayout(ctypes.Structure):
     _fields_ = [(n, ctypes.c_int64) for n in (
         "cov3d", "xys", "depths", "radii", "conics", "comp", "nth", "opac_eff", "records", "tile_count", "tile_bins",
-        "keys", "sorted_ids", "n_isect", "final_T", "final_idx", "l1_sign", "total")]
+        "keys", "sorted_ids", "n_isect", "final_T", "final_idx", "l1_sign", "stage_mask", "total")]
 
 
 _LAYOUTS = {}
@@ -412,6 +413,12 @@
 
 def _ws_view(ws, off, dtype, shape):
     return ws[off:off + math.prod(shape) * dtype.itemsize].view(dtype).view(shape)
+
+
+def _fwd_ppl(B):
+    ppl = c_int(0)
+    _lib.load().gol_raster_plan(c_int(B), ctypes.byref(ppl))
+    return ppl.value
 
 
 def _render_fwd_staged(B, N, src, attrs, background, with_depth, norm_lo, cap, ws, L, out_img, out_depth, alpha, depth_norm,
@@ -433,7 +440,7 @@
                        final_idx=a + L.final_idx, out_alpha=alpha, out_extra_norm=depth_norm, norm_lo=norm_lo,
                        l1_target=l1_target, l1_mask=l1_mask, l1_mask_c=l1_mask_c,
                        l1_sign=a + L.l1_sign if l1_target is not None else None, l1_partial=l1_partial, l1_out=l1_out,
-                       l1_scale=l1_scale)
+                       l1_scale=l1_scale, stage_mask=a + L.stage_mask)
 
 
 def _render_bwd_staged(B, N, src, attrs, grads, background, cap, ws, L, v_img, v_depth, v_alpha, use_l1, l1_mask, v_scale,
@@ -449,7 +456,7 @@
                        v_extra=field(9) if use_depth else None, v_opacity=field(3), grad_stride=GRAD_RECORD,
                        v_sign=a + L.l1_sign if use_l1 else None, v_sign_mask=l1_mask,
                        v_sign_mask_c=0 if l1_mask is None else l1_mask.shape[1], v_img_scale=v_scale,
-                       v_img_scale_mul=v_scale_mul)
+                       v_img_scale_mul=v_scale_mul, stage_mask=a + L.stage_mask, stage_mask_ppl=_fwd_ppl(B))
     if attrs is not None:
         means, scales, quats, opacity = attrs
         v_mean, v_scale_g, v_quat, v_opacity = grads
diff --git a/include/goliath_hip.h b/include/goliath_hip.h
--- a/include/goliath_hip.h
+++ b/include/goliath_hip.h
@@ -60,16 +60,16 @@
                       const float* background, float* out_img,
                       float* out_extra, float* final_Ts, int32_t* final_idx, float* out_alpha,
                       float* out_extra_norm, float norm_lo, const float* l1_target, const float* l1_mask, int l1_mask_c,
-                      uint8_t* l1_sign, float* l1_partial, float* l1_out, float l1_scale, int pixels_per_lane,
-                      void* stream);
+                      uint8_t* l1_sign, float* l1_partial, float* l1_out, float l1_scale, uint8_t* stage_mask,
+                      int pixels_per_lane, void* stream);
 int gol_rasterize_bwd(int B, int N, int img_h, int img_w, int block, int planar, const int32_t* tile_bins,
                       const int32_t* sorted_ids, int64_t capacity, const float* records, int with_extra,
                       const float* background, const float* final_Ts,
                       const int32_t* final_idx, const float* v_out_img, const float* v_out_extra,
                       const float* v_out_alpha, float* v_xy, float* v_conic, float* v_colors,
                       float* v_extra, float* v_opacity, int grad_stride, const uint8_t* v_sign, const float* v_sign_mask,
-                      int v_sign_mask_c, const float* v_img_scale, float v_img_scale_mul, int pixels_per_lane,
-                      void* stream);
+                      int v_sign_mask_c, const float* v_img_scale, float v_img_scale_mul, const uint8_t* stage_mask,
+                      int stage_mask_ppl, int pixels_per_lane, void* stream);
 int gol_raster_count_pairs(int B, int N, int img_h, int img_w, const int32_t* tile_bins, const int32_t* sorted_ids,
                            int64_t capacity, const float* records, const int32_t* final_idx, uint64_t* counts, void* stream);
 int gol_raster_plan(int B, int* fwd_pixels_per_lane);
@@ -86,7 +86,7 @@
 
 typedef struct gol_render_ws {
   int64_t cov3d, xys, depths, radii, conics, comp, nth, opac_eff, records, tile_count, tile_bins, keys, sorted_ids,
-      n_isect, final_T, final_idx, l1_sign, total;
+      n_isect, final_T, final_idx, l1_sign, stage_mask, total;
 } gol_render_ws;
 int gol_render_layout(int B, int N, int img_h, int img_w, int64_t capacity, int with_l1, gol_render_ws* layout);
 int gol_render_fwd(int B, int N, int img_h, int img_w, float glob_scale, float clip_thresh, const float* means,
```

Measured after the change: 3037 views/s (median of 6 runs). +1.2%, better.
